# holoskii/Rendering

Hardware: AMD Instinct MI355X
Metric: Mrays/s + ms/frame at 4096^2, 250k-tri BVH scene (higher is better)
Workload: dtype f32

## Files before the change

include/rtx_debug.h:

```cpp
#ifndef RTX_DEBUG_H
#define RTX_DEBUG_H
#include "rtx.h"
#ifdef __cplusplus
extern "C" {
#endif

int rtx_frame_mode(rtx_scene* scene, int* mode, float* split_ms, float* fused_ms);
int rtx_set_frame_mode(rtx_scene* scene, int mode);

int rtx_mesh_flatten_probe(const rtx_mesh* mesh, uint32_t* n_wide, void* wide_out, void* prune_out, uint32_t cap_wide, float* root_rec8);
int rtx_wide_node_slots(void);

int rtx_frame_mode_probe(int forced, int has_list, int fused_gave_up, uint32_t listed, uint32_t rule_tiles, int warm, const uint32_t* frame_samples2,
                         const float* frame_ms2, uint32_t frames_seen, int* mode, int* reprobe, int* probing);

int rtx_tile_list_probe(uint32_t width, uint32_t height, uint32_t band_height, uint32_t n_parts, uint32_t part, int halo, uint32_t row_begin, uint32_t row_end,
                        int strips, const uint32_t* rect4, uint32_t* out, size_t cap, size_t* need);

int rtx_views_plan_probe(uint32_t n_views, const uint32_t* sizes2, uint32_t* items3_out, size_t cap_items, size_t* n_items);

int rtx_source_p_probe(const float* tris9, uint32_t n, const double* S3, double sigma, int cam, float* out);

int rtx_cost_grid_read(rtx_scene* scene, uint32_t* out, size_t n, uint32_t* grid_w, uint32_t* grid_h);

int rtx_set_knob(rtx_scene* scene, const char* name, double value);

#define RTX_VARIANT_BOXES    1u
#define RTX_VARIANT_PLAIN    2u
#define RTX_VARIANT_ANALYTIC 4u
#define RTX_VARIANT_STATS    8u
#define RTX_VARIANT_CULL     16u
int rtx_kernel_variant(rtx_scene* scene, uint32_t* bits);

int rtx_ssaa_list_read(rtx_scene* scene, uint32_t* info, uint32_t* scan, size_t n);

int rtx_kernel_time_reset(rtx_scene* scene);
int rtx_kernel_time_stats(rtx_scene* scene, int which, uint32_t* launches, double* total_ms);

int rtx_tile_cost_read(rtx_scene* scene, uint32_t* out, size_t n);

int rtx_math_probe(int device, int op, uint32_t n, const float* x, const float* y, float* out);

int rtx_vec_probe(int device, int op, uint32_t n, const float* a, const float* b, float ior, float* out);

int rtx_desc_serialize(const rtx_scene_desc* desc, void* out, size_t cap, size_t* need);

int rtx_bvh_build_mode(int mode);
int rtx_bvh_launches(const rtx_bvh* bvh, uint32_t* launches, int* queued);

int rtx_scene_mesh_read(rtx_scene* scene, uint32_t mesh, uint32_t* counts2, float* node_bounds, int32_t* node_skip, int32_t* leaf_begin,
                        int32_t* leaf_count, uint32_t* refs);
int rtx_scene_mesh_flat_read(rtx_scene* scene, uint32_t mesh, uint32_t* n_wide, void* wide_out, void* prune_out, uint32_t cap_wide, float* root_rec8);
int rtx_scene_edit_times(rtx_scene* scene, float* ms4);
int rtx_scene_lights_read(rtx_scene* scene, uint32_t* n_lights, rtx_light* lights_out, uint32_t cap_lights, size_t* n_point_floats,
                          float* points_out, size_t cap_point_floats);
int rtx_scene_mesh_prune_copy_read(rtx_scene* scene, uint32_t mesh, uint32_t copy, uint32_t* n_copies, uint32_t* n_wide, void* prune_out,
                                   uint32_t cap_wide);
int rtx_scene_objects_read(rtx_scene* scene, uint32_t* n_objects, rtx_object* objects_out, uint32_t cap_objects, uint32_t* n_meshes);

int rtx_live_device_memory(size_t* allocations, size_t* bytes);

struct rtx_mesh_topology;
struct rtx_mesh_pose;
int rtx_place_probe(int device, const struct rtx_mesh_topology* topology, const float* pos, const float* nrm, const struct rtx_mesh_pose* pose,
                    float* tri24_out, float* lo_hi_out, uint32_t* flags_out);

#ifdef __cplusplus
}
#endif
#endif
```

rendering_amd/__init__.py:

```python
import ctypes as C
import os

import numpy as np

HERE = os.path.dirname(os.path.abspath(__file__))
ROOT = os.path.dirname(HERE)
LIB_RTX = os.path.join(HERE, "librtx_hip.so")
LIB_HOST = os.path.join(HERE, "librendering_host.so")

__all__ = ["load", "Scene", "Comm", "RtxError", "device_count", "math_probe", "gather_plan", "exported_symbols", "sphere_directions", "cube_cameras"]


class RtxError(RuntimeError):
    pass


class Counters(C.Structure):
    _fields_ = [("rays", C.c_uint64), ("box_tests", C.c_uint64), ("tri_tests", C.c_uint64), ("moot_rays", C.c_uint64)]


_rtx = None
_host = None

RTX_SYMBOLS = [
    "rtx_last_error", "rtx_device_count", "rtx_scene_create", "rtx_scene_destroy", "rtx_scene_set_view", "rtx_scene_bytes",
    "rtx_render_pass1", "rtx_sobel", "rtx_render_ssaa", "rtx_render_frame", "rtx_render_ac", "rtx_frame_status", "rtx_frame_mode", "rtx_set_frame_mode", "rtx_set_knob", "rtx_cost_grid_read", "rtx_mesh_flatten_probe", "rtx_wide_node_slots", "rtx_source_p_probe", "rtx_quantize_bgr8", "rtx_render_frame_host",
    "rtx_counters_enable", "rtx_counters_reset", "rtx_counters_read", "rtx_last_kernel_ms", "rtx_math_probe",
    "rtx_cast_rays", "rtx_trace_rays", "rtx_kernel_time_reset", "rtx_kernel_time_stats", "rtx_tile_cost_read", "rtx_set_row_ownership",
    "rtx_bvh_build", "rtx_bvh_info", "rtx_bvh_read", "rtx_bvh_destroy",
    "rtx_vec_probe", "rtx_desc_serialize", "rtx_bvh_build_mode", "rtx_bvh_launches", "rtx_comm_unique_id", "rtx_comm_create", "rtx_comm_info", "rtx_comm_destroy", "rtx_comm_agree", "rtx_gather", "rtx_gather_plan",
    "rtx_scene_mesh_read", "rtx_scene_mesh_flat_read", "rtx_scene_edit_times", "rtx_kernel_variant", "rtx_ssaa_list_read", "rtx_live_device_memory",
    "rtx_scene_lights_read", "rtx_scene_mesh_prune_copy_read", "rtx_scene_objects_read",
    "rtx_frame_mode_probe", "rtx_tile_list_probe", "rtx_place_probe",
    "rtx_views_plan_probe",
]

RTX_EDIT_SYMBOLS = ["rtx_scene_set_object", "rtx_scene_update_mesh", "rtx_scene_set_lights", "rtx_scene_set_objects"]

RTX_QUERY_SYMBOLS = ["rtx_occluded_rays"]

RTX_AOV_SYMBOLS = ["rtx_render_aov"]


RTX_AO_SYMBOLS = ["rtx_render_ao"]

RTX_SURFACE_SYMBOLS = ["rtx_surface_rays"]

RTX_LIGHT_SYMBOLS = ["rtx_light_rays"]

RTX_SCATTER_SYMBOLS = ["rtx_scatter_rays", "rtx_sky_rays"]

RTX_POINTS_SYMBOLS = ["rtx_light_points", "rtx_ao_points"]

RTX_DEFORM_SYMBOLS = ["rtx_scene_set_mesh_topology", "rtx_scene_deform_mesh"]

RTX_VIEWS_SYMBOLS = ["rtx_render_views"]


class MeshTopology(C.Structure):
    _fields_ = [(n, C.c_uint32) for n in ("n_tris", "n_pos", "n_nrm", "n_uv", "placed_pos", "placed_nrm")] + \
               [(n, C.c_void_p) for n in ("corner_pos", "corner_nrm", "corner_uv", "uv", "nrm")]


class MeshPose(C.Structure):
    _fields_ = [("pos", C.c_float * 3), ("rot_matrix", C.c_float * 16), ("size", C.c_float * 3), ("bias", C.c_float), ("ac_penalty", C.c_int32)]


class AovBuffers(C.Structure):
    _fields_ = [(n, C.c_void_p) for n in ("depth_dev", "object_dev", "triangle_dev", "uv_dev", "normal_dev", "albedo_dev")]


class SurfaceBuffers(C.Structure):
    _fields_ = [(n, C.c_void_p) for n in ("hits_dev", "position_dev", "normal_dev", "albedo_dev", "specular_dev")]


class LightBuffers(C.Structure):
    _fields_ = [("n_lights", C.c_uint32)] + [(n, C.c_void_p) for n in ("hits_dev", "diffuse_dev", "specular_dev", "light_diffuse_dev",
                                                                       "light_specular_dev", "light_open_dev")]


class ScatterBuffers(C.Structure):
    _fields_ = [(n, C.c_void_p) for n in ("hits_dev", "local_dev", "reflect_dev", "refract_dev", "weight_dev", "kinds_dev")]


class ViewTarget(C.Structure):
    _fields_ = [("width", C.c_uint32), ("height", C.c_uint32), ("cam_pos", C.c_float * 3), ("cam_matrix", C.c_float * 16),
                ("scale", C.c_float), ("aspect", C.c_float), ("fb_dev", C.c_void_p), ("mask_dev", C.c_void_p)]


def cube_cameras(pos):
    p = tuple(float(x) for x in np.asarray(pos, np.float32).reshape(3))
    return [(p, rot, 90.0) for rot in ((0.0, 90.0, 0.0), (0.0, -90.0, 0.0), (-90.0, 0.0, 0.0), (90.0, 0.0, 0.0), (0.0, 180.0, 0.0), (0.0, 0.0, 0.0))]


def views_plan_probe(sizes):
    rtx, _ = load()
    sz = np.ascontiguousarray(np.asarray(sizes, np.uint32).reshape(-1, 2))
    n = C.c_size_t(0)
    _check(rtx.rtx_views_plan_probe(sz.shape[0], _np_ptr(sz), None, 0, C.byref(n)), "rtx_views_plan_probe")
    out = np.zeros((n.value, 3), np.uint32)
    _check(rtx.rtx_views_plan_probe(sz.shape[0], _np_ptr(sz), _np_ptr(out), n.value, C.byref(n)), "rtx_views_plan_probe")
    return out


class AoParams(C.Structure):
    _fields_ = [("n_dirs", C.c_uint32), ("dirs_dev", C.c_void_p), ("radius", C.c_float)]


def sphere_directions(n):
    n = int(n)
    if n < 2 or n % 2:
        raise ValueError("sphere_directions: n must be even and at least 2, got %d" % n)
    i = np.arange(n // 2, dtype=np.float64) + 0.5
    z = 1.0 - 2.0 * i / n
    phi = i * (np.pi * (3.0 - np.sqrt(5.0)))
    r = np.sqrt(1.0 - z * z)
    half = np.stack([r * np.cos(phi), r * np.sin(phi), z], 1).astype(np.float32)
    return np.concatenate([half, -half], 0)


def load():
    global _rtx, _host
    if _rtx is not None:
        return _rtx, _host
    for p in (LIB_RTX, LIB_HOST):
        if not os.path.exists(p):
            raise RtxError("native library %s is missing -- build it with ./build.sh (hipcc, gfx950); "
                           "there is no CPU fallback" % p)
    try:
        import torch
    except Exception:
        pass
    rtx = C.CDLL(LIB_RTX, mode=C.RTLD_GLOBAL)
    host = C.CDLL(LIB_HOST, mode=C.RTLD_GLOBAL)
    rtx.rtx_last_error.restype = C.c_char_p
    vp, u32, i32 = C.c_void_p, C.c_uint32, C.c_int
    rtx.rtx_device_count.argtypes = [C.POINTER(C.c_int)]
    rtx.rtx_render_pass1.argtypes = [vp, u32, u32, vp, vp]
    rtx.rtx_sobel.argtypes = [vp, vp, u32, u32, vp, vp]
    rtx.rtx_render_ssaa.argtypes = [vp, vp, u32, u32, vp, vp]
    rtx.rtx_render_frame.argtypes = [vp, u32, u32, vp, vp, vp]
    rtx.rtx_render_ac.argtypes = [vp, vp, vp, vp]
    rtx.rtx_frame_status.argtypes = [vp, C.POINTER(C.c_uint32)]
    rtx.rtx_set_frame_mode.argtypes = [vp, C.c_int]
    rtx.rtx_set_knob.argtypes = [vp, C.c_char_p, C.c_double]
    rtx.rtx_cost_grid_read.argtypes = [vp, vp, C.c_size_t, C.POINTER(C.c_uint32), C.POINTER(C.c_uint32)]
    rtx.rtx_mesh_flatten_probe.argtypes = [vp, C.POINTER(C.c_uint32), vp, vp, C.c_uint32, vp]
    rtx.rtx_source_p_probe.argtypes = [vp, u32, vp, C.c_double, i32, vp]
    rtx.rtx_frame_mode_probe.argtypes = [i32, i32, i32, u32, u32, i32, vp, vp, u32, C.POINTER(i32), C.POINTER(i32), C.POINTER(i32)]
    rtx.rtx_tile_list_probe.argtypes = [u32, u32, u32, u32, u32, i32, u32, u32, i32, vp, vp, C.c_size_t, C.POINTER(C.c_size_t)]
    rtx.rtx_frame_mode.argtypes = [vp, C.POINTER(C.c_int), C.POINTER(C.c_float), C.POINTER(C.c_float)]
    rtx.rtx_quantize_bgr8.argtypes = [vp, vp, vp, vp]
    rtx.rtx_render_frame_host.argtypes = [vp, i32, vp]
    rtx.rtx_counters_enable.argtypes = [vp, i32]
    rtx.rtx_counters_reset.argtypes = [vp]
    rtx.rtx_counters_read.argtypes = [vp, C.POINTER(Counters)]
    rtx.rtx_last_kernel_ms.argtypes = [vp, i32, C.POINTER(C.c_float)]
    rtx.rtx_math_probe.argtypes = [i32, i32, u32, vp, vp, vp]
    rtx.rtx_cast_rays.argtypes = [vp, u32, vp, vp, vp]
    rtx.rtx_trace_rays.argtypes = [vp, u32, vp, vp, vp, vp]
    rtx.rtx_occluded_rays.argtypes = [vp, u32, vp, vp, vp, vp]
    rtx.rtx_render_aov.argtypes = [vp, u32, u32, C.POINTER(AovBuffers), vp]
    rtx.rtx_render_ao.argtypes = [vp, u32, u32, C.POINTER(AoParams), vp, vp, vp]
    rtx.rtx_surface_rays.argtypes = [vp, u32, vp, C.POINTER(SurfaceBuffers), vp]
    if hasattr(rtx, "rtx_light_rays"):
        rtx.rtx_light_rays.argtypes = [vp, u32, vp, C.POINTER(LightBuffers), vp]
    if hasattr(rtx, "rtx_scatter_rays"):
        rtx.rtx_scatter_rays.argtypes = [vp, u32, vp, C.POINTER(ScatterBuffers), vp]
        rtx.rtx_sky_rays.argtypes = [vp, u32, vp, vp, vp]
    if hasattr(rtx, "rtx_light_points"):
        rtx.rtx_light_points.argtypes = [vp, u32, vp, vp, C.POINTER(LightBuffers), vp]
        rtx.rtx_ao_points.argtypes = [vp, u32, vp, C.POINTER(AoParams), vp, vp, vp]
    if hasattr(rtx, "rtx_render_views"):
        rtx.rtx_render_views.argtypes = [vp, u32, C.POINTER(ViewTarget), i32, vp]
        rtx.rtx_views_plan_probe.argtypes = [u32, vp, vp, C.c_size_t, C.POINTER(C.c_size_t)]
        host.rah_view_target.argtypes = [vp, vp, vp, C.c_float, i32, i32, C.POINTER(ViewTarget)]
    rtx.rtx_kernel_time_reset.argtypes = [vp]
    rtx.rtx_kernel_time_stats.argtypes = [vp, i32, C.POINTER(C.c_uint32), C.POINTER(C.c_double)]
    rtx.rtx_tile_cost_read.argtypes = [vp, vp, C.c_size_t]
    rtx.rtx_set_row_ownership.argtypes = [vp, u32, u32, u32, i32]
    rtx.rtx_bvh_build.argtypes = [vp, u32, vp, vp, C.c_int32, i32, C.POINTER(vp)]
    rtx.rtx_bvh_info.argtypes = [vp, C.POINTER(u32), C.POINTER(u32), C.POINTER(u32), C.POINTER(C.c_float)]
    rtx.rtx_bvh_launches.argtypes = [vp, C.POINTER(u32), C.POINTER(C.c_int)]
    rtx.rtx_bvh_read.argtypes = [vp, vp, vp, vp, vp, vp]
    rtx.rtx_bvh_destroy.argtypes = [vp]
    rtx.rtx_bvh_destroy.restype = None
    rtx.rtx_scene_bytes.argtypes = [vp, C.POINTER(C.c_size_t)]
    rtx.rtx_vec_probe.argtypes = [i32, i32, u32, vp, vp, C.c_float, vp]
    rtx.rtx_comm_unique_id.argtypes = [vp]
    rtx.rtx_comm_create.argtypes = [vp, i32, i32, i32, C.POINTER(vp)]
    rtx.rtx_comm_info.argtypes = [vp, C.POINTER(C.c_int), C.POINTER(C.c_int)]
    rtx.rtx_comm_destroy.argtypes = [vp]
    rtx.rtx_comm_agree.argtypes = [vp, C.c_int, C.POINTER(C.c_int), vp]
    rtx.rtx_comm_destroy.restype = None
    rtx.rtx_gather.argtypes = [vp, vp, vp, C.c_size_t, i32, i32, vp]
    rtx.rtx_gather_plan.argtypes = [u32, u32, u32, C.c_size_t, i32, u32, vp, vp, vp, C.POINTER(u32)]
    host.rah_set_ac_build.argtypes = [i32, i32]
    host.rah_set_ac_build.restype = None
    host.rah_set_ac_build_device.argtypes = [i32]
    host.rah_set_ac_build_device.restype = None
    host.rah_bvh_build_info.argtypes = [vp, i32, C.POINTER(C.c_int), C.POINTER(C.c_float)]
    host.rah_last_error.restype = C.c_char_p
    host.rah_scene_load.restype = vp
    host.rah_scene_load.argtypes = [C.c_char_p, C.c_char_p, i32, i32]
    host.rah_scene_free.argtypes = [vp]
    host.rah_scene_dims.argtypes = [vp] + [C.POINTER(C.c_int)] * 4
    host.rah_scene_resize.argtypes = [vp, i32, i32]
    host.rah_scene_set_device.argtypes = [vp, i32]
    host.rah_set_flag.argtypes = [vp, C.c_char_p, i32]
    host.rah_flatten.restype = vp
    host.rah_flatten.argtypes = [vp]
    host.rah_flat_desc.restype = vp
    host.rah_flat_desc.argtypes = [vp]
    host.rah_flat_free.argtypes = [vp]
    host.rah_bvh_counts.argtypes = [vp, i32, vp]
    host.rah_scene_gpu.restype = vp
    host.rah_scene_gpu.argtypes = [vp]
    host.rah_render_host.argtypes = [vp, vp, i32]
    host.rah_save_bmp.argtypes = [vp, vp, C.c_char_p]
    host.rah_bvh_dump.argtypes = [vp, i32, vp, vp, vp, vp, vp]
    host.rah_tris.argtypes = [vp, i32, vp]
    host.rah_camera.argtypes = [vp, vp, vp, vp, vp]
    host.rah_scene_digest.argtypes = [vp, vp, i32]
    host.rah_view_flags.argtypes = [vp]
    if hasattr(host, "rah_max_ray_depth"):
        host.rah_max_ray_depth.argtypes = [vp]
    host.rah_load_bmp.argtypes = [C.c_char_p, C.POINTER(C.c_int), C.POINTER(C.c_int), vp, i32]
    host.rah_object_move.argtypes = [vp, i32] + [vp] * 5
    host.rah_object_type.argtypes = [vp, i32]
    host.rah_object_move_times.argtypes = [vp, vp]
    rtx.rtx_scene_set_object.argtypes = [vp, C.c_uint32, vp]
    rtx.rtx_scene_update_mesh.argtypes = [vp, C.c_uint32, vp, vp, vp, vp, vp, i32, vp]
    rtx.rtx_scene_mesh_read.argtypes = [vp, C.c_uint32] + [vp] * 6
    rtx.rtx_scene_mesh_flat_read.argtypes = [vp, C.c_uint32, vp, vp, vp, C.c_uint32, vp]
    rtx.rtx_scene_edit_times.argtypes = [vp, vp]
    rtx.rtx_kernel_variant.argtypes = [vp, C.POINTER(C.c_uint32)]
    rtx.rtx_ssaa_list_read.argtypes = [vp, vp, vp, C.c_size_t]
    rtx.rtx_live_device_memory.argtypes = [C.POINTER(C.c_size_t), C.POINTER(C.c_size_t)]
    rtx.rtx_scene_set_lights.argtypes = [vp, C.c_uint32, vp]
    rtx.rtx_scene_lights_read.argtypes = [vp, C.POINTER(C.c_uint32), vp, C.c_uint32, C.POINTER(C.c_size_t), vp, C.c_size_t]
    rtx.rtx_scene_mesh_prune_copy_read.argtypes = [vp, C.c_uint32, C.c_uint32, C.POINTER(C.c_uint32), C.POINTER(C.c_uint32), vp, C.c_uint32]
# ... 220 lines not shown


class RtxView(C.Structure):
    _fields_ = [("width", C.c_uint32), ("height", C.c_uint32), ("bias", C.c_float), ("max_ray_depth", C.c_int32), ("background", C.c_float * 3),
                ("flags", C.c_uint32), ("cam_pos", C.c_float * 3), ("cam_matrix", C.c_float * 16), ("scale", C.c_float), ("aspect", C.c_float)]


class RtxSceneDesc(C.Structure):
    _fields_ = [("view", RtxView), ("n_objects", C.c_uint32), ("objects", C.POINTER(RtxObject)), ("n_meshes", C.c_uint32),
                ("meshes", C.POINTER(_RtxMesh)), ("n_lights", C.c_uint32), ("lights", C.POINTER(RtxLight)), ("sky_w", C.c_uint32), ("sky_h", C.c_uint32),
                ("sky", C.c_void_p * 6)]


class RtxMeshBuild(C.Structure):
    _fields_ = [("tri_pos_dev", C.c_void_p), ("tri_nrm_dev", C.c_void_p), ("tri_tb_dev", C.c_void_p), ("root_lo", C.c_float * 3),
                ("root_hi", C.c_float * 3), ("ac_penalty", C.c_int32)]


class RtxMeshSource(C.Structure):
    _fields_ = [("keep", C.c_int32), ("mesh", C.POINTER(_RtxMesh)), ("build", C.POINTER(RtxMeshBuild))]


def mesh_flatten_probe(bvh):
    rtx, _ = load()
    bounds = np.ascontiguousarray(bvh["bounds"], np.float32); skip = np.ascontiguousarray(bvh["skip"], np.int32)
    lb = np.ascontiguousarray(bvh["leaf_begin"], np.int32); lc = np.ascontiguousarray(bvh["leaf_count"], np.int32)
    refs = np.ascontiguousarray(bvh["refs"], np.uint32); pos = np.ascontiguousarray(bvh["tris"][:, 0:9], np.float32)
    m = _RtxMesh()
    m.n_nodes, m.n_refs, m.n_tris = len(skip), len(refs), len(pos)
    m.node_bounds, m.node_skip, m.leaf_begin, m.leaf_count = bounds.ctypes.data, skip.ctypes.data, lb.ctypes.data, lc.ctypes.data
    m.refs, m.tri_pos = refs.ctypes.data, pos.ctypes.data
    n = C.c_uint32(0)
    root = np.zeros(8, np.float32)
    _check(rtx.rtx_mesh_flatten_probe(C.byref(m), C.byref(n), None, None, 0, _np_ptr(root)), "rtx_mesh_flatten_probe")
    S = int(rtx.rtx_wide_node_slots())
    wide = np.zeros((n.value, S, 8), np.float32); prune = np.zeros((n.value, 2 * S, 8), np.float32)
    _check(rtx.rtx_mesh_flatten_probe(C.byref(m), C.byref(n), _np_ptr(wide), _np_ptr(prune), n.value, _np_ptr(root)), "rtx_mesh_flatten_probe")
    return wide, prune[:, 0:S], prune[:, S:2 * S], root


def source_p_probe(v0, e1, e2, S, sigma, cam):
    rtx, _ = load()
    t = np.ascontiguousarray(np.concatenate([v0, e1, e2], 1), np.float32)
    S = np.ascontiguousarray(S, np.float64)
    out = np.zeros(len(t), np.float32)
    _check(rtx.rtx_source_p_probe(_np_ptr(t), len(t), _np_ptr(S), float(sigma), 1 if cam else 0, _np_ptr(out)), "rtx_source_p_probe")
    return out


def frame_mode_probe(forced, has_list, fused_gave_up, listed, rule_tiles, warm, frame_samples, frame_ms, frames_seen):
    rtx, _ = load()
    n = np.ascontiguousarray(frame_samples, np.uint32); ms = np.ascontiguousarray(frame_ms, np.float32)
    assert n.shape == (2,) and ms.shape == (2,)
    mode, reprobe, probing = C.c_int(-1), C.c_int(-1), C.c_int(-1)
    _check(rtx.rtx_frame_mode_probe(int(forced), int(has_list), int(fused_gave_up), int(listed), int(rule_tiles), int(warm), _np_ptr(n), _np_ptr(ms),
                                    int(frames_seen), C.byref(mode), C.byref(reprobe), C.byref(probing)), "rtx_frame_mode_probe")
    return mode.value, bool(reprobe.value), bool(probing.value)


def tile_list_probe(width, height, ownership, rows, strips, rect):
    rtx, _ = load()
    r = np.ascontiguousarray(rect, np.uint32)
    assert r.shape == (4,)
    args = [int(width), int(height)] + [int(x) for x in ownership] + [int(rows[0]), int(rows[1]), 1 if strips else 0, _np_ptr(r)]
    need = C.c_size_t(0)
    _check(rtx.rtx_tile_list_probe(*args, None, 0, C.byref(need)), "rtx_tile_list_probe")
    out = np.zeros(need.value, np.uint32)
    _check(rtx.rtx_tile_list_probe(*args, _np_ptr(out), out.size, C.byref(need)), "rtx_tile_list_probe")
    return out


def math_probe(op, x, y=None, device=0):
    rtx, _ = load()
    x = np.ascontiguousarray(x, np.float32)
    out = np.zeros_like(x)
    yp = None
    if y is not None:
        y = np.ascontiguousarray(np.broadcast_to(np.asarray(y, np.float32), x.shape))
        yp = _np_ptr(y)
    _check(rtx.rtx_math_probe(device, op, x.size, _np_ptr(x), yp, _np_ptr(out)), "rtx_math_probe")
    return out


def vec_probe(op, a, b=None, ior=1.0, device=0):
    rtx, _ = load()
    a = np.ascontiguousarray(a, np.float32).reshape(-1, 3)
    out = np.zeros_like(a)
    bp = None
    if b is not None:
        b = np.ascontiguousarray(b, np.float32).reshape(-1, 3)
        bp = _np_ptr(b)
    _check(rtx.rtx_vec_probe(device, op, a.shape[0], _np_ptr(a), bp, ior, _np_ptr(out)), "rtx_vec_probe")
    return out


def euler_matrix(rot):
    _, host = load()
    r = np.ascontiguousarray(np.asarray(rot, np.float32).reshape(3))
    m = np.zeros((4, 4), np.float32)
    host.rah_euler_matrix(_np_ptr(r), _np_ptr(m))
    return m


def place_probe(topology, stored_normals, vertices, normals, pose, device=-1):
    rtx, _ = load()
    f32 = lambda a, cols: np.ascontiguousarray(np.asarray(a, np.float32).reshape(-1, cols))
    cp = np.ascontiguousarray(topology["corner_pos"], np.uint32).reshape(-1, 3)
    cn = np.ascontiguousarray(topology["corner_nrm"], np.int32).reshape(-1, 3)
    cu = np.ascontiguousarray(topology["corner_uv"], np.int32).reshape(-1, 3)
    uv, sn, P = f32(topology["uv"], 2), f32(stored_normals, 3), f32(vertices, 3)
    N = f32(normals, 3) if normals is not None else None
    if N is not None and N.shape != sn.shape:
        raise ValueError("place_probe: normals must have the stored normals' shape %s, got %s" % (sn.shape, N.shape))
    nt = cp.shape[0]
    t = MeshTopology(nt, P.shape[0], sn.shape[0], uv.shape[0], int(topology["placed_pos"]), int(topology["placed_nrm"]),
                     cp.ctypes.data, cn.ctypes.data, cu.ctypes.data, uv.ctypes.data if uv.size else None, sn.ctypes.data if sn.size else None)
    ps = MeshPose()
    ps.pos[:] = [float(x) for x in np.asarray(pose["pos"], np.float32)]
    ps.size[:] = [float(x) for x in np.asarray(pose["size"], np.float32)]
    ps.rot_matrix[:] = [float(x) for x in euler_matrix(pose["rot"]).reshape(-1)]
    ps.bias = float(pose["bias"]); ps.ac_penalty = int(pose["ac_penalty"])
    tri = np.zeros(max(nt, 1) * 24, np.float32)
    lo_hi = np.zeros(12, np.float32)
    flags = np.zeros(2, np.uint32)
    _check(rtx.rtx_place_probe(device, C.byref(t), _np_ptr(P), _np_ptr(N) if N is not None else None, C.byref(ps), _np_ptr(tri), _np_ptr(lo_hi), _np_ptr(flags)),
           "rtx_place_probe")
    return dict(pos=tri[:nt * 9].reshape(nt, 9).copy(), nrm=tri[nt * 9:nt * 18].reshape(nt, 9).copy(), tb=tri[nt * 18:nt * 24].reshape(nt, 6).copy(),
                obj_lo=lo_hi[0:3].copy(), obj_hi=lo_hi[3:6].copy(), root_lo=lo_hi[6:9].copy(), root_hi=lo_hi[9:12].copy(),
                bad_input=bool(flags[0]), bad_placed=bool(flags[1]))


class Scene:

    def __init__(self, scene_path, width=-1, height=-1, device=0, cwd=ROOT):
        self.rtx, self.host = load()
        self.host.rah_set_ac_build_device(device)
        self.h = C.c_void_p(self.host.rah_scene_load(cwd.encode(), scene_path.encode(), width, height))
        if not self.h:
            raise RtxError("could not load scene %s: %s" % (scene_path, self.host.rah_last_error().decode(errors="replace")))
        self.device = device
        self._cwd = cwd
        self.host.rah_scene_set_device(self.h, device)
        self._dims()
        self._gpu = None

    def _dims(self):
        w, h, no, nl = C.c_int(), C.c_int(), C.c_int(), C.c_int()
        self.host.rah_scene_dims(self.h, C.byref(w), C.byref(h), C.byref(no), C.byref(nl))
        self.width, self.height, self.n_objects, self.n_lights = w.value, h.value, no.value, nl.value

    def close(self):
        if self.h:
            self.host.rah_scene_free(self.h)
            self.h = None
            self._gpu = None

    def resize(self, width, height):
        self.host.rah_scene_resize(self.h, width, height)
        self._dims()

    def camera_pose(self):
        pos, rot = np.zeros(3, np.float32), np.zeros(3, np.float32)
        self.host.rah_camera_get.argtypes = [C.c_void_p] * 3
        self.host.rah_camera_get(self.h, _np_ptr(pos), _np_ptr(rot))
        return pos, rot

# ... 734 lines not shown
```

rendering_amd/csrc/rtx_api.hip:

```cpp
#include <hip/hip_runtime.h>

#include <cstdio>
#include <dlfcn.h>
#include <algorithm>
#include <array>
#include <functional>
#include <cmath>
#include <cstring>
#include <memory>
#include <string>
#include <type_traits>
#include <vector>

#include "../../include/rtx.h"
#include "../../include/rtx_debug.h"
#include "../../include/rtx_scene_edit.h"
#include "../../include/rtx_query.h"
#include "../../include/rtx_aov.h"
#include "../../include/rtx_ao.h"
#include "../../include/rtx_surface.h"
#include "../../include/rtx_light.h"
#include "../../include/rtx_scatter.h"
#include "../../include/rtx_points.h"
#include "../../include/rtx_views.h"
// ... 588 lines not shown
	HIPCHK(fixed.upload(m.diffuse_map, (size_t)m.diffuse_w * m.diffuse_h * 3, &dm.diffuse));
	HIPCHK(fixed.upload(m.normal_map, (size_t)m.normal_w * m.normal_h * 3, &dm.normal));
	HIPCHK(fixed.upload(m.specular_map, (size_t)m.specular_w * m.specular_h, &dm.specular));
	dm.dW = m.diffuse_w; dm.dH = m.diffuse_h; dm.nW = m.normal_w; dm.nH = m.normal_h; dm.sW = m.specular_w; dm.sH = m.specular_h;
	return RTX_OK;
}

int uploadMesh(rtx_scene* s, const rtx_mesh& m, uint32_t mi, uint32_t nLights, DevBag& owned, DevBag& fixed, Mesh& dm, rtx_scene::SrcMesh& sm,
               rtx_scene::MeshLeaves& leaves, float bounds[6])
{
	memset(&dm, 0, sizeof(dm));
	int rc;
	if ((rc = uploadMeshGeometry(s, m, mi, nLights, owned, dm, sm, leaves, bounds))) return rc;
	HIPCHK(owned.upload(m.tri_nrm, (size_t)m.n_tris * 9, &dm.nrm));
	HIPCHK(owned.upload(m.tri_tb, m.tri_tb ? (size_t)m.n_tris * 6 : 0, &dm.tb));
	return uploadMeshFixed(m, fixed, dm);
}

int checkObjects(uint32_t n, const rtx_object* objects, uint32_t nMeshes)
{
	if (n && !objects) return fail(RTX_ERR_ARG, "objects is NULL");
	for (uint32_t i = 0; i < n; i++) {
		const rtx_object& o = objects[i];
		if (o.type < RTX_OBJ_SPHERE || o.type > RTX_OBJ_MESH) return fail(RTX_ERR_ARG, "bad object type");
		if (o.material < 0 || o.material > 3) return fail(RTX_ERR_ARG, "bad material");
		if (o.type == RTX_OBJ_MESH && (o.mesh < 0 || (uint32_t)o.mesh >= nMeshes)) return fail(RTX_ERR_ARG, "bad mesh index");
	}
	return RTX_OK;
}

std::vector<Object> objectRecords(uint32_t n, const rtx_object* objects, const std::vector<Mesh>& meshes, const std::vector<rtx_scene::SrcMesh>& sms,
                                  const std::vector<float>& meshBounds)
{
	std::vector<Object> objs(n);
	for (uint32_t i = 0; i < n; i++) {
		const rtx_object& o = objects[i];
		Object& d = objs[i];
		memset(&d, 0, sizeof(d));
		d.type = o.type; d.material = o.material;
		memcpy(d.pos, o.pos, 12); memcpy(d.color, o.color, 12); memcpy(d.normal, o.normal, 12);
		d.ior = o.ior; d.ambient = o.ambient; d.diffuse = o.diffuse; d.specular = o.specular; d.nSpecular = o.n_specular;
		d.r2 = o.radius2; d.mesh = o.mesh;
		if (o.type == RTX_OBJ_MESH) meshObjectRecord(&meshBounds[(size_t)o.mesh * 6], d, meshes[o.mesh], sms[o.mesh]);
	}
	return objs;
}

int uploadRecords(const std::vector<Mesh>& meshes, const std::vector<Object>& objs, const std::vector<float>& sb, DevBag& bag, const Mesh** devMeshes,
                  const Object** devObjs, const float** devSpheres)
{
	HIPCHK(bag.upload(sb.data(), sb.size(), devSpheres));
	HIPCHK(bag.upload(meshes.data(), meshes.size(), devMeshes));
	HIPCHK(bag.upload(objs.data(), objs.size(), devObjs));
	return RTX_OK;
}

void chooseAnalytic(rtx_scene* s)
{
	s->analytic = true;
	for (const Object& d : s->objectRecs) if (d.type == RTX_OBJ_MESH) s->analytic = false;
}

int checkLights(uint32_t n, const rtx_light* lights)
{
	if (n && !lights) return fail(RTX_ERR_ARG, "lights is NULL");
	for (uint32_t i = 0; i < n; i++) {
		const rtx_light& l = lights[i];
		if (l.type < RTX_LIGHT_DISTANT || l.type > RTX_LIGHT_AREA) return fail(RTX_ERR_ARG, "bad light type");
		if (l.type == RTX_LIGHT_AREA && (!l.points || l.n_points == 0)) return fail(RTX_ERR_ARG, "area light without sample points");
	}
	return RTX_OK;
}

int uploadLights(uint32_t n, const rtx_light* lights, DevBag& bag, std::vector<Light>& recs, const Light** dev)
{
	recs.resize(n);
	for (uint32_t i = 0; i < n; i++) {
		const rtx_light& l = lights[i];
		Light& d = recs[i];
		memset(&d, 0, sizeof(d));
		d.type = l.type; memcpy(d.color, l.color, 12); d.intensity = l.intensity;
		memcpy(d.dir, l.dir, 12); memcpy(d.pos, l.pos, 12);
		d.nPoints = l.n_points;
		if (l.type == RTX_LIGHT_AREA) HIPCHK(bag.upload(l.points, (size_t)l.n_points * 3, &d.points));
	}
	HIPCHK(bag.upload(recs.data(), recs.size(), dev));
	return RTX_OK;
}

void deriveLights(rtx_scene* s, uint32_t n, const rtx_light* lights)
{
	s->srcLightPos.clear(); s->srcLightIsPoint.clear(); s->estLights.clear();
	for (uint32_t i = 0; i < n; i++) {
		const rtx_light& l = lights[i];
		s->srcLightPos.push_back({ { l.pos[0], l.pos[1], l.pos[2] } });
		s->srcLightIsPoint.push_back(l.type == RTX_LIGHT_POINT ? 1 : 0);
		if (l.type == RTX_LIGHT_POINT) s->estLights.push_back({ { l.pos[0], l.pos[1], l.pos[2], 2.0f } });
		else if (l.type == RTX_LIGHT_DISTANT) s->estLights.push_back({ { l.dir[0], l.dir[1], l.dir[2], 1.0f } });
		else if (l.type == RTX_LIGHT_AREA) s->estLights.push_back({ { l.pos[0], l.pos[1], l.pos[2], 2.0f + 4.0f * (float)std::min<uint32_t>(l.n_points, 4096u) } });
	}
	s->params.nLights = n;
	s->params.nSrcLights = s->knobs.sources ? std::min<uint32_t>(n, kMaxSrcLights) : 0u;
}

void choosePlain(rtx_scene* s)
{
	s->plain = true;
	for (const Object& d : s->objectRecs) if (d.material != 0) s->plain = false;
	for (const Light& l : s->lightRecs) if (l.type == RTX_LIGHT_AREA) s->plain = false;
}

std::vector<float> analyticEstimate(rtx_scene* s, const rtx_object* objects, size_t n)
{
	std::vector<float> sb;
	s->estPlanes.clear();
	s->srcNmax = 1.0f;
	for (size_t i = 0; i < n; i++) {
		const rtx_object& o = objects[i];
		if (o.type == RTX_OBJ_PLANE) {
			s->estPlanes.push_back({ { o.pos[0], o.pos[1], o.pos[2], o.normal[0], o.normal[1], o.normal[2] } });
			const double nl = std::sqrt((double)o.normal[0] * o.normal[0] + (double)o.normal[1] * o.normal[1] + (double)o.normal[2] * o.normal[2]);
			if (!(nl <= 1e30)) s->srcNmax = INFINITY; else s->srcNmax = std::max(s->srcNmax, (float)(nl * 1.000001));
		}
		if (o.type != RTX_OBJ_SPHERE || !(o.radius2 > 0) || !std::isfinite(o.radius2)) continue;
		const float r = std::sqrt(o.radius2), w = (o.material == 1 || o.material == 2) ? 4000.0f : 300.0f;
		sb.insert(sb.end(), { o.pos[0] - r, o.pos[1] - r, o.pos[2] - r, o.pos[0] + r, o.pos[1] + r, o.pos[2] + r, w, 0.0f });
	}
	s->params.srcNmax2 = s->srcNmax * s->srcNmax * 1.00001f;
	return sb;
}

}

extern "C" {

const char* rtx_last_error(void) { return gErr.c_str(); }

int rtx_device_count(int* count)
{
	if (!count) return fail(RTX_ERR_ARG, "count is NULL");
	*count = 0;
	int n = 0;
	hipError_t e = hipGetDeviceCount(&n);
	if (e != hipSuccess) return fail(RTX_ERR_NO_DEVICE, std::string("hipGetDeviceCount: ") + hipGetErrorString(e));
	*count = n;
	return RTX_OK;
}

int rtx_scene_create(const rtx_scene_desc* desc, int device, rtx_scene** out)
{
	if (!desc || !out) return fail(RTX_ERR_ARG, "desc/out is NULL");
	*out = nullptr;
	int n = 0;
	if (hipGetDeviceCount(&n) != hipSuccess || n <= 0) return fail(RTX_ERR_NO_DEVICE, "no HIP device visible");
	if (device < 0 || device >= n) return fail(RTX_ERR_ARG, "device index out of range");
	HIPCHK(hipSetDevice(device));
	hipDeviceProp_t prop;
	HIPCHK(hipGetDeviceProperties(&prop, device));

	std::unique_ptr<rtx_scene, void (*)(rtx_scene*)> hold(new rtx_scene, rtx_scene_destroy);
	rtx_scene* s = hold.get();
	readKnobs(s->knobs);
	s->tileQueues.reserve(16);
	s->device = device;
	s->numCUs = prop.multiProcessorCount;
	memset(&s->params, 0, sizeof(Params));
// ... 1358 lines not shown

int rtx_views_plan_probe(uint32_t n_views, const uint32_t* sizes2, uint32_t* items3_out, size_t cap_items, size_t* n_items)
{
	if (!n_items || (n_views && !sizes2)) return fail(RTX_ERR_ARG, "rtx_views_plan_probe: NULL argument");
	uint64_t items = 0;
	if (int rc = checkViewSizes(n_views, sizes2, sizes2 + 1, 8, &items)) return rc;
	*n_items = (size_t)items;
	if (!items3_out || cap_items < items) return RTX_OK;
	std::vector<uint32_t> first(n_views + 1, 0u);
	for (uint32_t v = 0; v < n_views; v++) first[v + 1] = first[v] + (uint32_t)rtxviews::tilesOf(sizes2[2 * v], sizes2[2 * v + 1]);
	for (uint32_t item = 0; item < (uint32_t)items; item++) {
		const uint32_t v = rtxviews::viewOfItem([&](uint32_t i) { return first[i]; }, n_views, item);
		const rtxviews::Tile t = rtxviews::tileOfItem(item, first[v], rtxviews::tilesAcross(sizes2[2 * v]));
		items3_out[3 * (size_t)item] = v; items3_out[3 * (size_t)item + 1] = t.tx; items3_out[3 * (size_t)item + 2] = t.ty;
	}
	return RTX_OK;
}

int rtx_render_views(rtx_scene* s, uint32_t n_views, const rtx_view_target* views, int with_ssaa, void* stream)
{
	RoctxRange range("Render views (rtx_render_views)");
	if (!s) return fail(RTX_ERR_ARG, "scene is NULL");
	if (n_views == 0) return RTX_OK;
	if (!views) return fail(RTX_ERR_ARG, "rtx_render_views: views is NULL");
	uint64_t items64 = 0;
	if (int rc = checkViewSizes(n_views, &views[0].width, &views[0].height, sizeof(rtx_view_target), &items64)) return rc;
	for (uint32_t i = 0; i < n_views; i++) {
		if (!views[i].fb_dev) return fail(RTX_ERR_ARG, "rtx_render_views: view " + std::to_string(i) + " has no framebuffer (fb_dev is NULL)");
		if (with_ssaa && !views[i].mask_dev) return fail(RTX_ERR_ARG, "rtx_render_views: view " + std::to_string(i) + " has no mask (mask_dev is NULL) and SSAA is asked for");
	}
	if (s->params.bandH && s->params.nParts > 1) return fail(RTX_ERR_ARG, "rtx_render_views: the rows are shared among devices (rtx_set_row_ownership); deal out views, not rows");
	if (s->stats) return fail(RTX_ERR_UNSUPPORTED, "rtx_render_views collects no statistics (rtx_counters_enable)");
	if (showNormals(s)) return fail(RTX_ERR_UNSUPPORTED, "rtx_render_views does not render the normals view (RTX_FLAG_SHOW_NORMALS)");
	const uint32_t nItems = (uint32_t)items64;
	int rc = ensureWork(s);
	if (rc) return rc;
	hipStream_t st = (hipStream_t)stream;
	if ((rc = renderOn(s, st))) return rc;
	const size_t recBytes = (size_t)n_views * sizeof(ViewRec), tableBytes = recBytes + ((size_t)n_views + 1) * sizeof(uint32_t);
	HIPCHK(s->viewsTable.reserve(tableBytes));
	HIPCHK(s->viewsWork.reserve(64));
	if (with_ssaa) { HIPCHK(s->viewsItemView.reserve(nItems)); HIPCHK(s->viewsList.reserve((size_t)nItems * 64)); }
	if (s->viewsStagePending) { HIPCHK(hipEventSynchronize(s->viewsStaged)); s->viewsStagePending = false; }
	HIPCHK(s->viewsStage.reserve(tableBytes));
	ViewRec* recs = (ViewRec*)s->viewsStage.host();
	uint32_t* first = (uint32_t*)(s->viewsStage.host() + recBytes);
	uint32_t at = 0;
	for (uint32_t i = 0; i < n_views; i++) {
		const rtx_view_target& t = views[i];
		ViewRec& r = recs[i];
		r.width = t.width; r.height = t.height; r.scale = t.scale; r.aspect = t.aspect;
		memcpy(r.camPos, t.cam_pos, 12); memcpy(r.camM, t.cam_matrix, 64);
		r.firstItem = first[i] = at;
		r.fb = t.fb_dev; r.mask = t.mask_dev;
		r.tilesX = rtxviews::tilesAcross(t.width); r.pad[0] = r.pad[1] = r.pad[2] = 0;
		at += (uint32_t)rtxviews::tilesOf(t.width, t.height);
	}
	first[n_views] = at;
	HIPCHK(hipMemcpyAsync(s->viewsTable.get(), s->viewsStage.host(), tableBytes, hipMemcpyHostToDevice, st));
	HIPCHK(s->viewsStaged.create(hipEventDisableTiming));
	HIPCHK(hipEventRecord(s->viewsStaged, st));
	s->viewsStagePending = true;
	HIPCHK(hipMemsetAsync(s->viewsWork.get(), 0, 64 * sizeof(uint32_t), st));
	ViewsKernArgs k;
	k.P = s->params;
	k.A.views = (const ViewRec*)s->viewsTable.get(); k.A.first = (const uint32_t*)(s->viewsTable.get() + recBytes);
	k.A.nViews = n_views; k.A.nItems = nItems;
	k.A.itemView = s->viewsItemView; k.A.list = s->viewsList; k.A.heads = s->viewsWork;
	const Variant v = variantOf(s);
	const uint32_t itemBlocks = (nItems + 3) / 4;
	hipLaunchKernelGGL(viewsPass1Kernel(v), dim3(std::min<uint32_t>((uint32_t)s->blocksPass1, itemBlocks)), dim3(256), 0, st, k);
	HIPCHK(hipGetLastError());
	if (!with_ssaa) return RTX_OK;
	hipLaunchKernelGGL(rtxViewsMaskKernel, dim3(itemBlocks), dim3(256), 0, st, k.A);
	HIPCHK(hipGetLastError());
	k.P.frames = s->frames + s->framesArea;
	hipLaunchKernelGGL(viewsSsaaKernel(v), dim3(std::min<uint32_t>((uint32_t)s->blocksSsaa, nItems)), dim3(256), 0, st, k);
	HIPCHK(hipGetLastError());
	return RTX_OK;
}

int rtx_math_probe(int device, int op, uint32_t n, const float* x, const float* y, float* out)
{
	if (!x || !out || op < 0 || op > 4) return fail(RTX_ERR_ARG, "bad argument");
	int cnt = 0;
	if (hipGetDeviceCount(&cnt) != hipSuccess || cnt <= 0) return fail(RTX_ERR_NO_DEVICE, "no HIP device visible");
	HIPCHK(hipSetDevice(device));
	DevArray<float> dx, dy, dout;
	const size_t bytes = (size_t)n * sizeof(float);
	HIPCHK(dx.reserve(n)); HIPCHK(dy.reserve(n)); HIPCHK(dout.reserve(n));
	HIPCHK(hipMemcpy(dx, x, bytes, hipMemcpyHostToDevice));
	if (y) HIPCHK(hipMemcpy(dy, y, bytes, hipMemcpyHostToDevice));
	else HIPCHK(hipMemset(dy, 0, bytes));
	hipLaunchKernelGGL(rtxMathProbeKernel, dim3((n + 255) / 256), dim3(256), 0, nullptr, op, n, (const float*)dx, (const float*)dy, dout.get());
	HIPCHK(hipGetLastError());
	HIPCHK(hipMemcpy(out, dout, bytes, hipMemcpyDeviceToHost));
	return RTX_OK;
}

int rtx_vec_probe(int device, int op, uint32_t n, const float* a, const float* b, float ior, float* out)
{
	if (!a || !out || op < 0 || op > 3 || (op < 3 && !b)) return fail(RTX_ERR_ARG, "bad argument");
	int cnt = 0;
	if (hipGetDeviceCount(&cnt) != hipSuccess || cnt <= 0) return fail(RTX_ERR_NO_DEVICE, "no HIP device visible");
	HIPCHK(hipSetDevice(device));
	DevArray<float> da, db, dout;
	const size_t bytes = (size_t)n * 3 * sizeof(float);
	HIPCHK(da.reserve((size_t)n * 3)); HIPCHK(dout.reserve((size_t)n * 3));
	HIPCHK(hipMemcpy(da, a, bytes, hipMemcpyHostToDevice));
	if (b) { HIPCHK(db.reserve((size_t)n * 3)); HIPCHK(hipMemcpy(db, b, bytes, hipMemcpyHostToDevice)); }
	hipLaunchKernelGGL(rtxVecProbeKernel, dim3((n + 255) / 256), dim3(256), 0, nullptr, op, n, (const float*)da, (const float*)db, ior, dout.get());
	HIPCHK(hipGetLastError());
	HIPCHK(hipMemcpy(out, dout, bytes, hipMemcpyDeviceToHost));
	return RTX_OK;
}

}

#include "rtx_comm.hip"

#include "rtx_edit.hip"

#include "rtx_deform.hip"
```

rendering_amd/csrc/rtx_device.h:

```cpp
#pragma once
#include <stdint.h>

namespace rtxd {

struct Node {
	float b[6];
	int32_t link;
	int32_t first;
};
static_assert(sizeof(Node) == 32, "node must be one s_load_dwordx8");

constexpr int kWideLevels = 3;
constexpr int kWideSlots = 1 << kWideLevels;
constexpr int kWideStackEntries = 72;
struct WideNode { Node slot[kWideSlots]; };
static_assert(kWideSlots == 8 && sizeof(WideNode) == 32 * kWideSlots, "wide node = eight slots, two s_load_dwordx16 per four");

struct RefA { float v0x, v0y, v0z; uint32_t tri; };
struct RefB { float e1x, e1y, e1z, e2x; };
struct RefC { float e2y, e2z; };
static_assert(sizeof(RefA) == 16 && sizeof(RefB) == 16 && sizeof(RefC) == 8, "reference records = dwordx4 + dwordx4 + dwordx2");

struct PruneRec { float c[3]; float P; float h[3]; float Pgen; };
static_assert(sizeof(PruneRec) == 32, "prune record = two dwordx4");
constexpr uint32_t kMaxSrcLights = 6;
constexpr float kSrcAinfMax = 32.0f;
struct PlaneRec { float qc[3]; float wlo; float qr[3]; float whi; };
static_assert(sizeof(PlaneRec) == 32, "plane record = two dwordx4");
struct PruneBlock { PruneRec box[kWideSlots]; PlaneRec plane[kWideSlots]; };
static_assert(sizeof(PruneBlock) == 64 * kWideSlots, "prune block");

struct Mesh {
	const Node* nodes;
	const RefA* refA;
	const RefB* refB;
	const RefC* refC;
	const float* nrm;
	const float* uv;
	const float* tb;
	const float* diffuse;
	const float* normal;
	const float* specular;
	uint32_t nNodes, nRefs, nTris;
	uint32_t dW, dH, nW, nH, sW, sH;
	uint32_t boxesRegular;
	const struct WideNode* wide;
	uint32_t nWide, padw;
	const PruneBlock* prune;
	float vmax, padv;
	PruneRec rootRec;
	float fatRadius, centre[3], radius;
};

struct Object {
	int32_t type, material;
	float pos[3];
	float r2;
	float normal[3];
	int32_t mesh;
	float color[3];
	float ior, ambient, diffuse, specular, nSpecular;
	float rootBox[6];
	float fatRadius, centre[3], radius;
	uint32_t meshFlags;
	uint32_t pad[2];
	const Node* nodes; const RefA* refA; const RefB* refB; const RefC* refC; const struct WideNode* wide; const struct PruneBlock* prune;
	uint32_t nNodes; float vmax;
	uint32_t pruneBoxes;
	uint32_t srcStride;
};
static_assert(sizeof(Object) == 192, "object record = three 64-byte lines");

struct Light {
	int32_t type;
	float color[3];
	float intensity;
	float dir[3];
	float pos[3];
	uint32_t nPoints;
	const float* points;
	uint32_t pad[2];
};
static_assert(sizeof(Light) == 64, "light record = one 64-byte line");

struct View {
	uint32_t width, height;
	float bias;
	int32_t maxDepth;
	float bg[3];
	uint32_t flags;
	float camPos[3];
	float camM[16];
	float scale, aspect;
};

struct Params {
	View view;
	const Object* objects;
	const Mesh* meshes;
	const Light* lights;
	const float* const* sky;
	uint32_t nObjects, nLights, skyW, skyH;
	uint32_t rowBegin, rowEnd;
	uint32_t tilesX, tileRow0, nTiles;
	uint32_t bandH, nParts, part, halo;
	uint32_t* workCounter;
	const uint32_t* tileList;
	uint32_t tilesY, pad3;
	const uint8_t* ssaaMask;
	const uint32_t* ssaaPixels;
	const uint32_t* ssaaScan;
	uint32_t* tileCost;
	uint32_t tilesXFull, pad2;
	float* frames;
	uint32_t totalLanes;
	uint32_t nSrcLights;
	float* fb;
	const float* probeRays;
	float* probeHits;
	float* probeColours;
	uint32_t nProbe;
	float srcNmax2;
	unsigned long long* counters;
	uint32_t* tileReady;
	uint32_t* tileSobel;
	const uint8_t* tileNeed;
	unsigned long long* tileFlags;
	unsigned long long* ssaaQueue;
	unsigned long long* frameCtl;
	const uint32_t* countExpect;
	const uint32_t* splitLimits;
	uint8_t* maskOut;
	uint32_t listedTiles, epoch, queueCap, veryBudget, tilesYFull, heavyTicks, stripBit, padF1;
};

constexpr int kFrameFields = 14;

}
```

rendering_amd/csrc/rtx_kernels.hip:

```cpp
#include <hip/hip_runtime.h>
#include <stdint.h>

#include "rtx_device.h"
#include "rtx_tuning.h"

#pragma clang fp contract(off)

using namespace rtxd;

constexpr uint32_t kPopNum = 1u, kPopDen = 2u;

namespace {

#if RTX_DBG
#define RTX_DBG_ONLY(...) __VA_ARGS__
#else
#define RTX_DBG_ONLY(...)
#endif
#if RTX_DBG || RTX_WAVE_TRACE
#define RTX_TRACE_ONLY(...) __VA_ARGS__
#else
#define RTX_TRACE_ONLY(...)
#endif

// ... 199 lines not shown
	uint64_t ki = (uint64_t)__double_as_longlong(kd);
	kd -= 0x1.8p+47;
	double rr = ylogx - kd;
	uint64_t t = powTab[32 + ki % 32];
	t += (ki + signBias) << (52 - 5);
	double s = __longlong_as_double((long long)t);
	double zz = __builtin_fma(0x1.c6af84b912394p-5, rr, 0x1.ebfce50fac4f3p-3);
	double rr2 = rr * rr;
	double yv = __builtin_fma(0x1.62e42ff0c52d6p-1, rr, 1.0);
	yv = __builtin_fma(zz, rr2, yv);
	yv = yv * s;
	return (float)yv;
}

__device__ __forceinline__ V3 reflectDir(V3 d, V3 n) { float k = 2 * dot(d, n); return d - n * k; }

__device__ __forceinline__ V3 refractDir(V3 d, V3 n, float ior)
{
	float n1 = 1, n2 = ior;
	float cosi = clampRef(-1, 1, dot(d, n));
	V3 mn = n;
	if (cosi < 0) cosi = -cosi;
	else { float t = n1; n1 = n2; n2 = t; mn = -n; }
	float rri = n1 / n2;
	float k = 1 - rri * rri * (1 - cosi * cosi);
	if (k < 0) return mk(0, 0, 0);
	return d * rri + mn * (rri * cosi - __builtin_sqrtf(k));
}

__device__ __forceinline__ float fresnelKr(V3 d, V3 n, float ior)
{
	float n1 = 1, n2 = ior;
	float cosi = clampRef(-1, 1, dot(d, n));
	if (cosi > 0) { float t = n1; n1 = n2; n2 = t; }
	float sint = n1 / n2 * __builtin_sqrtf(fmaxRef(0.f, 1 - cosi * cosi));
	if (sint >= 1) return 1;
	float cost = __builtin_sqrtf(fmaxRef(0.f, 1 - sint * sint));
	cosi = fabsf(cosi);
	float rs = ((n2 * cosi) - (n1 * cost)) / ((n2 * cosi) + (n1 * cost));
	float rp = ((n1 * cosi) - (n2 * cost)) / ((n1 * cosi) + (n2 * cost));
	return (rs * rs + rp * rp) / 2;
}

__device__ __forceinline__ int toPixel(float v, int mx)
{
	int val = (int)((v + 1.0f) / 2.0f * mx);
	if (val >= mx) val = mx - 1;
	if (val < 0) val = 0;
	return val;
}
__device__ __forceinline__ V3 load3(const float* p) { return mk(p[0], p[1], p[2]); }
typedef const __attribute__((address_space(1))) float* GlobalFloats;
__device__ __forceinline__ GlobalFloats inGlobal(const float* p) { return (GlobalFloats)(uintptr_t)p; }
__device__ __forceinline__ V3 load3(GlobalFloats p) { return mk(p[0], p[1], p[2]); }

__device__ __noinline__ V3 skyFetch(const float* const* sky, int W, int H, V3 dir)
{
	float ax = fabsf(dir.x), ay = fabsf(dir.y), az = fabsf(dir.z);
	float m = fmaxRef(ax, fmaxRef(ay, az));
	V3 a; int face, i, j;
	if (m == az) {
		if (dir.z < 0) { a = dir * (1 / -dir.z); face = 1; i = toPixel(a.y, H); j = toPixel(a.x, W); }
		else { a = dir * (1 / dir.z); face = 3; i = toPixel(a.y, H); j = toPixel(-a.x, W); }
	}
	else if (m == ax) {
		if (dir.x < 0) { a = dir * (1 / -dir.x); face = 0; i = toPixel(a.y, H); j = toPixel(-a.z, W); }
		else { a = dir * (1 / dir.x); face = 2; i = toPixel(a.y, H); j = toPixel(a.z, W); }
	}
	else {
		if (dir.y < 0) { a = dir * (1 / -dir.y); face = 5; i = toPixel(a.z, H); j = toPixel(a.x, W); }
		else { a = dir * (1 / dir.y); face = 4; i = toPixel(a.z, H); j = toPixel(a.x, W); }
	}
	return load3(inGlobal(sky[face]) + ((size_t)i * W + j) * 3);
}

__device__ __forceinline__ V3 skyColor(const Params& P, V3 dir)
{
	if (!(P.view.flags & 2u)) return mk(P.view.bg[0], P.view.bg[1], P.view.bg[2]);
	return skyFetch(P.sky, (int)P.skyW, (int)P.skyH, dir);
}

__device__ __forceinline__ int texel(int dim, float coord) { int v = (int)(dim * coord); if (v >= dim) v = dim - 1; if (v < 0) v = 0; return v; }

__device__ __forceinline__ float attenuation(float intensity, float l2)
{
	return fminRef(1.0f, (float)((double)intensity / (4 * 3.14159265358979323846 * (double)l2 / 1000)));
}

struct Hit { int obj; float t; uint32_t tri; float u, v; };
RTX_TRACE_ONLY(__device__ unsigned long long gDbgWave[3 * 16384];)
RTX_DBG_ONLY(
__device__ unsigned long long gDbgTimeline[3 * 8192 * 160];
__device__ unsigned long long gDbgHist[64];
)
#if RTX_DBG >= 3
#define RTX_T0 const unsigned long long dbgB0 = __builtin_readcyclecounter();
#define RTX_ACC(k) { const unsigned long long dbgE = __builtin_readcyclecounter() - dbgB0; if (__lane_id() == (uint32_t)__ffsll((long long)ballot(true)) - 1u) { atomicAdd(&gDbgHist[16 + 2 * (k)], dbgE); atomicAdd(&gDbgHist[17 + 2 * (k)], 1ull); } }
#else
#define RTX_T0
#define RTX_ACC(k)
#endif
struct Counts { unsigned long long rays, box, tri, wNodes, wTri, wS2, wS3, wS4, wLeaves, wLeafSkips, wChunks, wChunkSkips, triLanes, moot, cNodes, cFilter, cExact,
                aWalks, sWalks, sVisits, sLeaves, sPasses, sExact; };

template <typename T> __device__ __forceinline__ T after(T x, uint32_t v)
{
	asm("" : "+s"(x) : "s"(v));
	return x;
}

__device__ __forceinline__ float waveMax(float v)
{
#define RTX_STEP(ctrl) "s_nop 1\n\tv_max_f32_dpp %0, %0, %0 " ctrl "\n\t"
	asm volatile(RTX_STEP("quad_perm:[1,0,3,2] row_mask:0xf bank_mask:0xf") RTX_STEP("quad_perm:[2,3,0,1] row_mask:0xf bank_mask:0xf")
	             RTX_STEP("row_half_mirror row_mask:0xf bank_mask:0xf") RTX_STEP("row_mirror row_mask:0xf bank_mask:0xf")
	             RTX_STEP("row_bcast:15 row_mask:0xa bank_mask:0xf") RTX_STEP("row_bcast:31 row_mask:0xc bank_mask:0xf")
	             "s_nop 0" : "+v"(v));
#undef RTX_STEP
	return __int_as_float(__builtin_amdgcn_readlane(__float_as_int(v), 63));
}

struct Bundle {
	float ocx, ocy, ocz, rox, roy, roz;
	float dcx, dcy, dcz, rdx, rdy, rdz;
	float kd;
	float roMax;
	float kdRoSum;
	float roRd;
	bool sane;
};
constexpr float kFilterK = 0x1p-18f;
constexpr float kFilterEta = 1e-30f;

__device__ __forceinline__ void centreRadius(float lo, float hi, float& c, float& r)
{
	c = unif(0.5f * (lo + hi));
	r = unif((0.5f * (hi - lo)) * (1.0f + 0x1p-19f) + 0x1p-21f * fmaxf(fabsf(lo), fabsf(hi)));
}

__device__ __forceinline__ void waveMaxMin(float v, float& hi, float& lo)
{
#define RTX_STEP(ctrl) "v_max_f32_dpp %0, %0, %0 " ctrl "\n\tv_min_f32_dpp %1, %1, %1 " ctrl "\n\ts_nop 0\n\t"
	asm volatile("s_nop 1\n\t"
		"v_max_f32_dpp %0, %2, %2 quad_perm:[1,0,3,2] row_mask:0xf bank_mask:0xf\n\tv_min_f32_dpp %1, %2, %2 quad_perm:[1,0,3,2] row_mask:0xf bank_mask:0xf\n\ts_nop 0\n\t"
		RTX_STEP("quad_perm:[2,3,0,1] row_mask:0xf bank_mask:0xf")
		RTX_STEP("row_half_mirror row_mask:0xf bank_mask:0xf") RTX_STEP("row_mirror row_mask:0xf bank_mask:0xf")
		RTX_STEP("row_bcast:15 row_mask:0xa bank_mask:0xf") RTX_STEP("row_bcast:31 row_mask:0xc bank_mask:0xf")
		"s_nop 0" : "=&v"(hi), "=&v"(lo) : "v"(v));
#undef RTX_STEP
	hi = __int_as_float(__builtin_amdgcn_readlane(__float_as_int(hi), 63));
	lo = __int_as_float(__builtin_amdgcn_readlane(__float_as_int(lo), 63));
}

__device__ __forceinline__ Bundle makeBundle(bool active, const V3& o, const V3& d, bool sameOrigin = false)
{
	const float qnan = __builtin_nanf("");
	Bundle B;
	float lo, hi;
#define RTX_RANGE(x, c, r) waveMaxMin(active ? (x) : qnan, hi, lo); centreRadius(lo, hi, c, r)
	if (sameOrigin) {
		const int first = __builtin_ctzll(ballot(active) | (1ull << 63));
		B.ocx = __int_as_float(__builtin_amdgcn_readlane(__float_as_int(o.x), first)); B.ocy = __int_as_float(__builtin_amdgcn_readlane(__float_as_int(o.y), first));
		B.ocz = __int_as_float(__builtin_amdgcn_readlane(__float_as_int(o.z), first));
		B.rox = B.roy = B.roz = 0.0f;
	}
	else {
		RTX_RANGE(o.x, B.ocx, B.rox); RTX_RANGE(o.y, B.ocy, B.roy); RTX_RANGE(o.z, B.ocz, B.roz);
	}
	RTX_RANGE(d.x, B.dcx, B.rdx); RTX_RANGE(d.y, B.dcy, B.rdy); RTX_RANGE(d.z, B.dcz, B.rdz);
// ... 48 lines not shown
	const float ax = B.ocx - ra.v0x, ay = B.ocy - ra.v0y, az = B.ocz - ra.v0z;
	const float s1 = fabsf(e1x) + fabsf(e1y) + fabsf(e1z), s2 = fabsf(e2x) + fabsf(e2y) + fabsf(e2z);
	const float wux = __builtin_fmaf(e2y, az, -(e2z * ay)), wuy = __builtin_fmaf(e2z, ax, -(e2x * az)), wuz = __builtin_fmaf(e2x, ay, -(e2y * ax));
	float nuc = __builtin_fmaf(B.dcz, wuz, __builtin_fmaf(B.dcy, wuy, B.dcx * wux));
	const float cux = __builtin_fmaf(B.dcy, e2z, -(B.dcz * e2y)), cuy = __builtin_fmaf(B.dcz, e2x, -(B.dcx * e2z)), cuz = __builtin_fmaf(B.dcx, e2y, -(B.dcy * e2x));
	const float nurO = __builtin_fmaf(B.roRd, s2, __builtin_fmaf(B.roz, fabsf(cuz), __builtin_fmaf(B.roy, fabsf(cuy), B.rox * fabsf(cux))));
	const float nur = (nurO + __builtin_fmaf(B.rdz, fabsf(wuz), __builtin_fmaf(B.rdy, fabsf(wuy), B.rdx * fabsf(wux)))) * (1.0f + 0x1p-19f);
	const float Eu = __builtin_fmaf(f.kda, s2, kFilterEta);
	if (!CULL) nuc *= f.sg;
	const float nuLo = nuc - nur - Eu;
	const uint64_t rejU = (ballot(nuc + nur < -Eu) | ballot(nuLo > f.detHi1)) & f.ok;
	if ((open & ~rejU) == 0) return rejU;
	const float wvx = __builtin_fmaf(ay, e1z, -(az * e1y)), wvy = __builtin_fmaf(az, e1x, -(ax * e1z)), wvz = __builtin_fmaf(ax, e1y, -(ay * e1x));
	float nvc = __builtin_fmaf(B.dcz, wvz, __builtin_fmaf(B.dcy, wvy, B.dcx * wvx));
	const float cvx = __builtin_fmaf(e1y, B.dcz, -(e1z * B.dcy)), cvy = __builtin_fmaf(e1z, B.dcx, -(e1x * B.dcz)), cvz = __builtin_fmaf(e1x, B.dcy, -(e1y * B.dcx));
	const float nvrO = __builtin_fmaf(B.roRd, s1, __builtin_fmaf(B.roz, fabsf(cvz), __builtin_fmaf(B.roy, fabsf(cvy), B.rox * fabsf(cvx))));
	const float nvr = (nvrO + __builtin_fmaf(B.rdz, fabsf(wvz), __builtin_fmaf(B.rdy, fabsf(wvy), B.rdx * fabsf(wvx)))) * (1.0f + 0x1p-19f);
	const float Ev = __builtin_fmaf(f.kda, s1, kFilterEta);
	if (!CULL) nvc *= f.sg;
	return rejU | ((ballot(nvc + nvr < -Ev) | ballot(nuLo + (nvc - nvr - Ev) > f.detHi1)) & f.ok);
}

template <bool CULL, bool STATS>
__device__ __forceinline__ void triTestOne(float v0x, float v0y, float v0z, float e1x, float e1y, float e1z, float e2x, float e2y, float e2z,
                                           uint32_t tri, const V3& o, const V3& d, float& bt, float& bu, float& bv, uint32_t& btri)
{
	const float px = d.y * e2z - d.z * e2y, py = d.z * e2x - d.x * e2z, pz = d.x * e2y - d.y * e2x;
	const float det = e1x * px + e1y * py + e1z * pz;
	if ((CULL ? det : fabsf(det)) < RTX_EPS8) return;
	const float tx = o.x - v0x, ty = o.y - v0y, tz = o.z - v0z;
	const float nu = tx * px + ty * py + tz * pz;
	if (CULL) {
		if (nu < -0x1p-20f || nu > det * (1.0f + 0x1p-20f)) return;
	}
	const float inv = 1 / det;
	const float u = nu * inv;
	if (u < 0 || u > 1) return;
	const float qx = ty * e1z - tz * e1y, qy = tz * e1x - tx * e1z, qz = tx * e1y - ty * e1x;
	const float v = (d.x * qx + d.y * qy + d.z * qz) * inv;
	if (v < 0 || u + v > 1) return;
	const float t = (e2x * qx + e2y * qy + e2z * qz) * inv;
	if (t < 0) return;
	if (t < bt) { bt = t; bu = u; bv = v; btri = tri; }
}

template <bool CULL>
__device__ __forceinline__ void triTestLane(const RefA& ra, const RefB& rb, const RefC& rc, float ox, float oy, float oz, float dx, float dy, float dz,
                                            float& t, float& u, float& v)
{
	const float e1x = rb.e1x, e1y = rb.e1y, e1z = rb.e1z, e2x = rb.e2x, e2y = rc.e2y, e2z = rc.e2z;
	const float px = dy * e2z - dz * e2y, py = dz * e2x - dx * e2z, pz = dx * e2y - dy * e2x;
	const float det = e1x * px + e1y * py + e1z * pz;
	if ((CULL ? det : fabsf(det)) < RTX_EPS8) return;
	const float tx = ox - ra.v0x, ty = oy - ra.v0y, tz = oz - ra.v0z;
	const float nu = tx * px + ty * py + tz * pz;
	if (CULL) { if (nu < -0x1p-20f || nu > det * (1.0f + 0x1p-20f)) return; }
	const float inv = 1 / det;
	const float uu = nu * inv;
	if (uu < 0 || uu > 1) return;
	const float qx = ty * e1z - tz * e1y, qy = tz * e1x - tx * e1z, qz = tx * e1y - ty * e1x;
	const float vv = (dx * qx + dy * qy + dz * qz) * inv;
	if (vv < 0 || uu + vv > 1) return;
	const float tt = (e2x * qx + e2y * qy + e2z * qz) * inv;
	if (tt < 0) return;
	t = tt; u = uu; v = vv;
}

#define RTX_LEAF_BATCH_MAX (RTX_LEAF_BATCH > RTX_LEAF_BATCH_FEW ? RTX_LEAF_BATCH : RTX_LEAF_BATCH_FEW)
struct LeafEntry { uint32_t start, count, first, pad0, maskLo, maskHi, pad1, pad2; };
typedef uint32_t u32x4v __attribute__((ext_vector_type(4)));
__shared__ LeafEntry leafBatch[4][RTX_LEAF_BATCH_MAX];
struct WideItem { int32_t link; uint32_t first, maskLo, maskHi; };
__shared__ WideItem wideStack[4][kWideStackEntries];
__shared__ float pruneUni[4][48];
constexpr float kPruneC = 216.0f;
__device__ __forceinline__ bool boxFailsRegular(float blox, float bhix, float bloy, float bhiy, float bloz, float bhiz, const V3& o, float ix, float iy, float iz)
{
	const float xlo = (blox - o.x) * ix, xhi = (bhix - o.x) * ix, ylo = (bloy - o.y) * iy, yhi = (bhiy - o.y) * iy;
	const float zlo = (bloz - o.z) * iz, zhi = (bhiz - o.z) * iz;
	float nx, ny, nz, fx, fy, fz, tn, tf;
	asm("v_min_f32 %0, %1, %2" : "=v"(nx) : "v"(xlo), "v"(xhi)); asm("v_max_f32 %0, %1, %2" : "=v"(fx) : "v"(xlo), "v"(xhi));
	asm("v_min_f32 %0, %1, %2" : "=v"(ny) : "v"(ylo), "v"(yhi)); asm("v_max_f32 %0, %1, %2" : "=v"(fy) : "v"(ylo), "v"(yhi));
	asm("v_min_f32 %0, %1, %2" : "=v"(nz) : "v"(zlo), "v"(zhi)); asm("v_max_f32 %0, %1, %2" : "=v"(fz) : "v"(zlo), "v"(zhi));
	asm("v_max3_f32 %0, %1, %2, %3" : "=v"(tn) : "v"(nx), "v"(ny), "v"(nz));
	asm("v_min3_f32 %0, %1, %2, %3" : "=v"(tf) : "v"(fx), "v"(fy), "v"(fz));
	return tn > tf;
}

__device__ __forceinline__ uint32_t pruneLaneK(const float* pu)
{
	const uint32_t lane = laneNow(), axis = lane & 3u;
	const uint32_t word = 2u * lane - axis;
	uint32_t ui = (lane >> 5) * 3u + axis;
	ui = ui < 5u ? ui : 5u;
	const uint32_t lds = (uint32_t)(uintptr_t)(const __attribute__((address_space(3))) float*)(pu + ui * 8u);
	return lds << 16 | word * 4u;
}
template <bool BOXES, bool CULL = true>
__device__ __forceinline__ uint32_t pruneEval8(const RTX_AS1 char* blk, const float* pu, float tmaxB, uint32_t laneK = 0)
{
	static_assert(kWideSlots == 8, "pruneEval8: lanes = 16 records x 4");
	const uint32_t off = laneK & 0xffffu;
	const float f0 = *(const RTX_AS1 float*)(blk + off), f1 = *(const RTX_AS1 float*)(blk + off + 16u);
	const __attribute__((address_space(3))) f4v* ur = (const __attribute__((address_space(3))) f4v*)(uintptr_t)(laneK >> 16);
	const f4v ua = ur[0], ub = ur[1];
	const float c = __uint_as_float(__float_as_uint(f0) ^ __float_as_uint(ub.x));
	const float ai = fmaxf(c - ua.z, ua.w - c) + f1;
	const float ax = fabsf(f0) + f1;
	const float dq = __builtin_fmaf(ua.y, ax, __builtin_fmaf(fabsf(ua.x), f1, ua.x * f0));
	const float oq = ua.z * f0;
	const float orr = __builtin_fmaf(ua.w, ax, fabsf(ua.z) * f1);
	const float pm = oq - orr, pp = oq + orr;
	float ainf, dqHi, oqLo, oqHi, w0, w1, t0, t1, t2, t3;
	asm volatile("s_nop 1\n\t"
	             "v_max_f32_dpp %6, %10, %10 quad_perm:[1,2,0,3] row_mask:0xf bank_mask:0xf\n\t"
	             "v_add_f32_dpp %7, %11, %11 quad_perm:[1,2,0,3] row_mask:0xf bank_mask:0xf\n\t"
	             "v_add_f32_dpp %8, %12, %12 quad_perm:[1,2,0,3] row_mask:0xf bank_mask:0xf\n\t"
	             "v_add_f32_dpp %9, %13, %13 quad_perm:[1,2,0,3] row_mask:0xf bank_mask:0xf\n\t"
	             "v_mov_b32_dpp %4, %14 quad_perm:[3,3,3,3] row_mask:0xf bank_mask:0xf\n\t"
	             "v_mov_b32_dpp %5, %15 quad_perm:[3,3,3,3] row_mask:0xf bank_mask:0xf\n\t"
	             "v_max_f32_dpp %0, %10, %6 quad_perm:[2,0,1,3] row_mask:0xf bank_mask:0xf\n\t"
	             "v_add_f32_dpp %1, %11, %7 quad_perm:[2,0,1,3] row_mask:0xf bank_mask:0xf\n\t"
	             "v_add_f32_dpp %2, %12, %8 quad_perm:[2,0,1,3] row_mask:0xf bank_mask:0xf\n\t"
	             "v_add_f32_dpp %3, %13, %9 quad_perm:[2,0,1,3] row_mask:0xf bank_mask:0xf"
	             : "=&v"(ainf), "=&v"(dqHi), "=&v"(oqLo), "=&v"(oqHi), "=&v"(w0), "=&v"(w1), "=&v"(t0), "=&v"(t1), "=&v"(t2), "=&v"(t3)
	             : "v"(ai), "v"(dq), "v"(pm), "v"(pp), "v"(f0), "v"(f1));
	const float detHi = dqHi + ub.x;
	const float ntHi = (w1 - oqLo) + ub.y, ntLo = (w0 - oqHi) - ub.y;
	uint64_t deadPlane;
	if (CULL) deadPlane = ballot(detHi < 0.0f) | ballot(ntHi < 0.0f) | (ballot(detHi > 0.0f) & ballot(ntLo >= tmaxB * (detHi * (1.0f + 0x1p-18f))));
	else {
		const float dql = __builtin_fmaf(-ua.y, ax, __builtin_fmaf(-fabsf(ua.x), f1, ua.x * f0));
		float dqLo;
		asm volatile("s_nop 1\n\t"
		             "v_add_f32_dpp %1, %2, %2 quad_perm:[1,2,0,3] row_mask:0xf bank_mask:0xf\n\t"
		             "s_nop 1\n\t"
		             "v_add_f32_dpp %0, %2, %1 quad_perm:[2,0,1,3] row_mask:0xf bank_mask:0xf"
		             : "=&v"(dqLo), "=&v"(t0) : "v"(dql));
		const float detLo = dqLo - ub.x;
		const uint64_t front = ballot(detLo > 0.0f), back = ballot(detHi < 0.0f);
		deadPlane = (front & (ballot(ntHi < 0.0f) | ballot(ntLo >= tmaxB * (detHi * (1.0f + 0x1p-18f))))) |
		            (back & (ballot(ntLo > 0.0f) | ballot(-ntHi >= tmaxB * (-detLo * (1.0f + 0x1p-18f)))));
	}
	uint32_t deadBits = (uint32_t)(deadPlane >> 32);
	if (BOXES) {
		const float Pn = ainf <= kSrcAinfMax ? w0 : w1;
		const float rho = __builtin_fmaf(ub.z * ainf, Pn, 0x1p-17f * (ainf + ub.w)) * (1.0f + 0x1p-20f) + 1e-30f;
		const float hh = f1 + rho;
		const float a = (c - hh) - ua.w, b = (c + hh) - ua.z;
		const float e = fminf(fminf(a * ua.x, a * ua.y), ub.y), f = fmaxf(fmaxf(b * ua.x, b * ua.y), -ub.y);
		float ent, ext;
		asm volatile("s_nop 1\n\t"
		             "v_max_f32_dpp %2, %4, %4 quad_perm:[1,2,0,3] row_mask:0xf bank_mask:0xf\n\t"
		             "v_min_f32_dpp %3, %5, %5 quad_perm:[1,2,0,3] row_mask:0xf bank_mask:0xf\n\t"
		             "s_nop 0\n\t"
		             "v_max_f32_dpp %0, %4, %2 quad_perm:[2,0,1,3] row_mask:0xf bank_mask:0xf\n\t"
		             "v_min_f32_dpp %1, %5, %3 quad_perm:[2,0,1,3] row_mask:0xf bank_mask:0xf"
		             : "=&v"(ent), "=&v"(ext), "=&v"(t0), "=&v"(t1) : "v"(e), "v"(f));
		const uint64_t deadBox = ballot(ent > ext) | ballot(ext < 0.0f) | ballot(ent > tmaxB * (1.0f + 0x1p-18f));
		deadBits |= (uint32_t)deadBox;
	}
	return ~deadBits & 0x11111111u;
}

template <bool STATS, bool CULL, bool REGULAR, bool WIDE = false, bool FEWRAYS = false, bool BOXES = true>
__device__ __forceinline__ void meshWalk(const u32x16& mp, const Bundle& B, bool consider, bool shadow, const V3& o, const V3& d,
                                         float ix, float iy, float iz, bool sx, bool sy, bool sz, float tLimit,
                                         float& bt, float& bu, float& bv, uint32_t& btri, Counts& cnt, uint32_t srcSel = 0)
{
#define RTX_MP(k) (((uint64_t)mp[2 * (k) + 1] << 32) | mp[2 * (k)])
	const Node* nodes = (const Node*)RTX_MP(0);
	const RTX_AS1 char* refA = (const RTX_AS1 char*)(uintptr_t)RTX_MP(1);
	const RTX_AS1 char* refB = (const RTX_AS1 char*)(uintptr_t)RTX_MP(2);
	const RTX_AS1 char* refC = (const RTX_AS1 char*)(uintptr_t)RTX_MP(3);
	const uint32_t nN = mp[12];
	bt = kFltMax; bu = 0; bv = 0; btri = 0;
	if (nN == 0) return;
	constexpr uint32_t kLeafBatch = FEWRAYS ? RTX_LEAF_BATCH_FEW : RTX_LEAF_BATCH;
	float tmaxB = unif(waveMax(consider ? tLimit : -__builtin_inff()));
	uint32_t resume = consider ? 0u : kNever;
	const uint32_t nRays4 = 4u * (uint32_t)__popcll(ballot(consider));
	uint32_t i = 0;
	const uint32_t last = nN - 1;
	u32x8 nd = sload8(nodes);
	LeafEntry* entries = leafBatch[threadIdx.x >> 6];
	WideItem* stack = wideStack[threadIdx.x >> 6];
	const WideNode* wideNodes = WIDE ? (const WideNode*)RTX_MP(4) : nullptr;
	uint32_t sp = 0;
	const RTX_AS1 char* pruneRecs = nullptr;
	float* pu = pruneUni[threadIdx.x >> 6];
	if (WIDE) {
		pruneRecs = (const RTX_AS1 char*)(uintptr_t)RTX_MP(5);
#undef RTX_MP
		if (pruneRecs != nullptr) {
			pruneRecs += (size_t)srcSel * mp[15] * sizeof(PruneBlock);
			const float dlx = B.dcx - B.rdx, dhx = B.dcx + B.rdx, dly = B.dcy - B.rdy, dhy = B.dcy + B.rdy, dlz = B.dcz - B.rdz, dhz = B.dcz + B.rdz;
			const float wide = 1.0f + 0x1p-21f, narrow = 1.0f - 0x1p-21f;
			float lx = __builtin_amdgcn_rcpf(dhx), hx = __builtin_amdgcn_rcpf(dlx);
			float ly = __builtin_amdgcn_rcpf(dhy), hy = __builtin_amdgcn_rcpf(dly), lz = __builtin_amdgcn_rcpf(dhz), hz = __builtin_amdgcn_rcpf(dlz);
			lx *= lx > 0 ? narrow : wide; hx *= hx > 0 ? wide : narrow;
			ly *= ly > 0 ? narrow : wide; hy *= hy > 0 ? wide : narrow;
			lz *= lz > 0 ? narrow : wide; hz *= hz > 0 ? wide : narrow;
			const bool usx = (dlx > 0x1p-100f || dhx < -0x1p-100f), usy = (dly > 0x1p-100f || dhy < -0x1p-100f), usz = (dlz > 0x1p-100f || dhz < -0x1p-100f);
			if (laneNow() == 0) {
				const bool nx = hx < 0, ny = hy < 0, nz = hz < 0;
				const bool okx = usx && (lx > 0 || nx), oky = usy && (ly > 0 || ny), okz = usz && (lz > 0 || nz);
				const float ilx = nx ? -hx : lx, ihx = nx ? -lx : hx, ily = ny ? -hy : ly, ihy = ny ? -ly : hy, ilz = nz ? -hz : lz, ihz = nz ? -lz : hz;
				const float ocx = nx ? -B.ocx : B.ocx, ocy = ny ? -B.ocy : B.ocy, ocz = nz ? -B.ocz : B.ocz;
				const float cap = B.kd * (kPruneC / kFilterK);
				const float omax = fmaxf(fmaxf(fabsf(B.ocx) + B.rox, fabsf(B.ocy) + B.roy), fabsf(B.ocz) + B.roz);
				const float eB = kFilterK * (omax + F(mp[13])) * (1.0f + 0x1p-20f) + 1e-30f;
				const float inf = __builtin_inff(), kd2 = 2.0f * B.kd;
				*(f4v*)(pu + 0) = f4v{ ilx, ihx, ocx - B.rox, ocx + B.rox };  *(f4v*)(pu + 4) = f4v{ __uint_as_float(nx ? 0x80000000u : 0u), okx ? inf : -inf, cap, omax };
				*(f4v*)(pu + 8) = f4v{ ily, ihy, ocy - B.roy, ocy + B.roy };  *(f4v*)(pu + 12) = f4v{ __uint_as_float(ny ? 0x80000000u : 0u), oky ? inf : -inf, cap, omax };
				*(f4v*)(pu + 16) = f4v{ ilz, ihz, ocz - B.roz, ocz + B.roz }; *(f4v*)(pu + 20) = f4v{ __uint_as_float(nz ? 0x80000000u : 0u), okz ? inf : -inf, cap, omax };
				float dcx = B.dcx, dcy = B.dcy, dcz = B.dcz, rdx = B.rdx, rdy = B.rdy, rdz = B.rdz;
				asm volatile("" : "+v"(dcx), "+v"(dcy), "+v"(dcz), "+v"(rdx), "+v"(rdy), "+v"(rdz));
				*(f4v*)(pu + 24) = f4v{ dcx, rdx, B.ocx, B.rox }; *(f4v*)(pu + 28) = f4v{ kd2, eB, 0.0f, 0.0f };
				*(f4v*)(pu + 32) = f4v{ dcy, rdy, B.ocy, B.roy }; *(f4v*)(pu + 36) = f4v{ kd2, eB, 0.0f, 0.0f };
				*(f4v*)(pu + 40) = f4v{ dcz, rdz, B.ocz, B.roz }; *(f4v*)(pu + 44) = f4v{ kd2, eB, 0.0f, 0.0f };
			}
			if (!B.sane) pruneRecs = nullptr;
		}
	}
	if (WIDE && RTX_DBG) { cnt.aWalks++; if (shadow) cnt.sWalks++; }
	uint32_t laneK = WIDE ? pruneLaneK(pu) : 0u;
	asm volatile("" : "+v"(laneK));
	if (WIDE) {
		const uint64_t m0 = ballot(consider);
		if (laneNow() == 0) { WideItem it; it.link = 1; it.first = 0; it.maskLo = (uint32_t)m0; it.maskHi = (uint32_t)(m0 >> 32); stack[0] = it; }
		sp = 1;
	}
	for (;;) {
		RTX_DBG_ONLY(const unsigned long long dbgP1 = __builtin_readcyclecounter();)
		uint32_t batch = 0, total = 0;
		uint32_t soleFirst = 0;
		uint32_t myReach = 0;
		if (WIDE) {
			const uint32_t lane = laneNow();
			const uint64_t openM = ballot(resume != kNever);
			auto noteLeaf = [&](int32_t link, uint32_t first, uint64_t m) {
				const bool in = ((((lane & 32u) ? (uint32_t)(m >> 32) : (uint32_t)m) >> (lane & 31u)) & 1u) != 0;
				const uint32_t n = (uint32_t)~link;
				if (RTX_DBG) { cnt.wLeaves++; if (shadow) cnt.sLeaves++; }
				if (m != 0 && n != 0) {
					if (kLeafBatch == 1 && !FEWRAYS) soleFirst = uni(first);
					else if (lane == 0) {
						LeafEntry en;
						en.first = first; en.count = n; en.maskLo = (uint32_t)m; en.maskHi = (uint32_t)(m >> 32); en.start = total; en.pad0 = en.pad1 = en.pad2 = 0;
						entries[batch] = en;
					}
					myReach |= in ? 1u << batch : 0u;
					batch = uni(batch + 1);
					total = uni(total + n);
				}
			};
#define RTX_PUSH(lnk, fst, m)                                                                                                  \
			{                                                                                                                  \
				if (lane == 0) { WideItem ni; ni.link = (int32_t)(lnk); ni.first = (fst); ni.maskLo = (uint32_t)(m); ni.maskHi = (uint32_t)((m) >> 32); stack[sp] = ni; } \
				sp = uni(sp + 1);                                                                                              \
			}
			while (sp != 0 && batch < kLeafBatch) {
				sp = uni(sp - 1);
				const WideItem it = stack[sp];
				const int32_t link = (int32_t)uni((uint32_t)it.link);
				const uint32_t itFirst = it.first;
				const uint32_t mlo = uni(it.maskLo), mhi = uni(it.maskHi);
				const uint64_t inM = ((uint64_t)mhi << 32 | mlo) & openM;
				if (link < 0) {
					noteLeaf(link, itFirst, inM);
					continue;
				}
				if (inM == 0) continue;
				if (RTX_DBG) { cnt.wNodes++; if (shadow) cnt.sVisits++; }
				const WideNode* w = wideNodes + (uint32_t)(link - 1);
				u32x16 wa = sload16(w), wb = sload16((const char*)w + 64);
				uint32_t aliveM = 0x11111111u;
				const bool evalPrune = pruneRecs != nullptr;
				if (evalPrune) {
					aliveM = pruneEval8<BOXES, CULL>(pruneRecs + ((size_t)(uint32_t)(link - 1) << 9), pu, tmaxB, laneK);
					if (RTX_DBG) { cnt.wS4++; cnt.wLeafSkips += (uint32_t)kWideSlots - (uint32_t)__popc(aliveM); }
				}
#define RTX_ALIVE(k) ((aliveM >> (4 * (k))) & 1u)
#define RTX_ALIVE4(q) ((aliveM >> (16 * (q))) & 0x1111u)
#define RTX_SLOT(rec, base, k)                                                                                                     \
				if ((int32_t)rec[base + 6] != 0 && RTX_ALIVE(k)) {                                                         \
					const bool fail = boxFailsRegular(F(rec[base]), F(rec[base + 1]), F(rec[base + 2]), F(rec[base + 3]), F(rec[base + 4]), F(rec[base + 5]), o, ix, iy, iz); \
					const uint64_t mk_ = ballot(!fail) & inM;                                                                       \
					if (RTX_DBG) cnt.wS3++;                                                                                         \
					if (mk_ != 0) RTX_PUSH(rec[base + 6], rec[base + 7], mk_)                                                       \
				}
				if (RTX_ALIVE4(1) != 0) {
#pragma unroll
					for (int q4 = kWideSlots / 4 - 1; q4 >= 1; --q4) {
						if (RTX_ALIVE4(q4) == 0) continue;
						const u32x16 wc = sload16((const char*)w + 128 * q4), wd = sload16((const char*)w + 128 * q4 + 64);
						RTX_SLOT(wd, 8, 4 * q4 + 3) RTX_SLOT(wd, 0, 4 * q4 + 2) RTX_SLOT(wc, 8, 4 * q4 + 1) RTX_SLOT(wc, 0, 4 * q4)
					}
					const char* w0 = (const char*)w;
					asm volatile("" : "+s"(w0));
					wa = sload16(w0); wb = sload16(w0 + 64);
				}
				if (RTX_ALIVE4(0) != 0) {
					RTX_SLOT(wb, 8, 3) RTX_SLOT(wb, 0, 2) RTX_SLOT(wa, 8, 1)
					if ((int32_t)wa[6] != 0 && RTX_ALIVE(0)) {
						const bool fail = boxFailsRegular(F(wa[0]), F(wa[1]), F(wa[2]), F(wa[3]), F(wa[4]), F(wa[5]), o, ix, iy, iz);
						const uint64_t mk_ = ballot(!fail) & inM;
						if (RTX_DBG) cnt.wS3++;
						if (mk_ != 0) {
							if ((int32_t)wa[6] < 0 && batch < kLeafBatch) noteLeaf((int32_t)wa[6], wa[7], mk_);
							else RTX_PUSH(wa[6], wa[7], mk_)
						}
					}
				}
#undef RTX_SLOT
#undef RTX_PUSH
#undef RTX_ALIVE
#undef RTX_ALIVE4
			}
		}
		else {
			while (i < nN && batch < kLeafBatch) {
				const int32_t link = (int32_t)nd[6];
				const uint32_t next = uni(i + 1);
				const uint32_t nxt = link > 0 ? (uint32_t)link : next;
				const Node* nb = after(nodes, nd[7]);
				const u32x8 nxA = sload8(nb + (next < last ? next : last));
				const u32x8 nxB = sload8(nb + (nxt < last ? nxt : last));
				const bool act = i >= resume;
				const float xlo = (F(nd[0]) - o.x) * ix, xhi = (F(nd[1]) - o.x) * ix, ylo = (F(nd[2]) - o.y) * iy, yhi = (F(nd[3]) - o.y) * iy;
				const float zlo = (F(nd[4]) - o.z) * iz, zhi = (F(nd[5]) - o.z) * iz;
				bool fail;
				if (REGULAR) {
					float nx, ny, nz, fx, fy, fz, tn, tf;
					asm("v_min_f32 %0, %1, %2" : "=v"(nx) : "v"(xlo), "v"(xhi)); asm("v_max_f32 %0, %1, %2" : "=v"(fx) : "v"(xlo), "v"(xhi));
					asm("v_min_f32 %0, %1, %2" : "=v"(ny) : "v"(ylo), "v"(yhi)); asm("v_max_f32 %0, %1, %2" : "=v"(fy) : "v"(ylo), "v"(yhi));
					asm("v_min_f32 %0, %1, %2" : "=v"(nz) : "v"(zlo), "v"(zhi)); asm("v_max_f32 %0, %1, %2" : "=v"(fz) : "v"(zlo), "v"(zhi));
					asm("v_max3_f32 %0, %1, %2, %3" : "=v"(tn) : "v"(nx), "v"(ny), "v"(nz));
					asm("v_min3_f32 %0, %1, %2, %3" : "=v"(tf) : "v"(fx), "v"(fy), "v"(fz));
					fail = tn > tf;
				}
				else {
					float tmin = sx ? xhi : xlo, tmx = sx ? xlo : xhi;
					const float tymin = sy ? yhi : ylo, tymax = sy ? ylo : yhi;
					fail = (tmin > tymax) || (tymin > tmx);
					if (tymin > tmin) tmin = tymin;
					if (tymax < tmx) tmx = tymax;
					const float tzmin = sz ? zhi : zlo, tzmax = sz ? zlo : zhi;
					fail = fail || (tmin > tzmax) || (tzmin > tmx);
				}
				const bool pass = act && !fail;
				if (act && fail) resume = nxt;
				if (STATS) cnt.box += __popcll(ballot(act));
				if (RTX_DBG) cnt.wNodes++;
				const uint64_t m = ballot(pass);
				if (m == 0) {
					nd = nxB;
					i = uni(nxt);
					continue;
				}
				if (link < 0) {
					const uint32_t n = (uint32_t)~link;
					if (STATS) cnt.tri += (unsigned long long)__popcll(m) * n;
					if (RTX_DBG) cnt.wLeaves++;
					if (n != 0) {
						if (kLeafBatch == 1 && !FEWRAYS) soleFirst = nd[7];
						else if (laneNow() == 0) {
							LeafEntry en;
							en.first = nd[7]; en.count = n; en.maskLo = (uint32_t)m; en.maskHi = (uint32_t)(m >> 32); en.start = total; en.pad0 = en.pad1 = en.pad2 = 0;
							entries[batch] = en;
						}
						myReach |= pass ? 1u << batch : 0u;
						batch = uni(batch + 1);
						total = uni(total + n);
					}
				}
				nd = nxA;
				i = next;
			}
		}
		const uint32_t lane = laneNow();
		RTX_DBG_ONLY(
		const unsigned long long dbgP2 = __builtin_readcyclecounter();
		cnt.cNodes += dbgP2 - dbgP1;
		unsigned long long dbgExact = 0;
		)
		uint32_t ecur = 0;
		auto assign = [&](uint32_t p0, uint32_t& r, uint32_t& myEnt) {
			r = 0; myEnt = 0;
// ... 23 lines not shown
			if (RTX_DBG) { cnt.wTri += __popcll(cand); if (shadow) cnt.sExact += __popcll(cand); if (cand == 0) cnt.wS2++; }
			if (cand == 0) return false;
			bool improved = false;
			RTX_DBG_ONLY(const unsigned long long dbgE0 = __builtin_readcyclecounter();)
			if (FEWRAYS && !STATS && nRays4 <= (uint32_t)__popcll(cand) * 3u) {
				const uint64_t raysOpen = ballot(resume != kNever);
				const uint32_t mLo = entries[myEnt].maskLo, mHi = entries[myEnt].maskHi;
				const bool isCand = ((cand >> lane) & 1ull) != 0;
				uint64_t rays = raysOpen;
				while (rays != 0) {
					const int r = __builtin_ctzll(rays);
					rays &= rays - 1;
#define RTX_RL(x) __int_as_float(__builtin_amdgcn_readlane(__float_as_int(x), r))
					const float rox = RTX_RL(o.x), roy = RTX_RL(o.y), roz = RTX_RL(o.z), rdx = RTX_RL(d.x), rdy = RTX_RL(d.y), rdz = RTX_RL(d.z);
					const float rbt = RTX_RL(bt);
#undef RTX_RL
					const bool reached = ((((uint32_t)r & 32u) ? mHi : mLo) >> ((uint32_t)r & 31u)) & 1u;
					float t = __builtin_inff(), u = 0, v = 0;
					if (isCand && reached) triTestLane<CULL>(ra, rb, rc, rox, roy, roz, rdx, rdy, rdz, t, u, v);
					const bool better = t < rbt;
					const float tmin = -waveMax(better ? -t : -__builtin_inff());
					const uint64_t at = ballot(better && t == tmin);
					if (at != 0) {
						const int w = __builtin_ctzll(at);
						const float wt = __int_as_float(__builtin_amdgcn_readlane(__float_as_int(t), w)), wu = __int_as_float(__builtin_amdgcn_readlane(__float_as_int(u), w));
						const float wv = __int_as_float(__builtin_amdgcn_readlane(__float_as_int(v), w));
						const uint32_t wtri = (uint32_t)__builtin_amdgcn_readlane((int)ra.tri, w);
						if (lane == (uint32_t)r) { bt = wt; bu = wu; bv = wv; btri = wtri; improved = true; }
					}
				}
				cand = 0;
			}
			const float btBefore = bt;
			while (cand != 0) {
				const int c = __builtin_ctzll(cand);
				cand &= cand - 1;
#define RTX_RL(x) __int_as_float(__builtin_amdgcn_ds_bpermute(c << 2, __float_as_int(x)))
				const float v0x = RTX_RL(ra.v0x), v0y = RTX_RL(ra.v0y), v0z = RTX_RL(ra.v0z);
				const float e1x = RTX_RL(rb.e1x), e1y = RTX_RL(rb.e1y), e1z = RTX_RL(rb.e1z);
				const float e2x = RTX_RL(rb.e2x), e2y = RTX_RL(rc.e2y), e2z = RTX_RL(rc.e2z);
#undef RTX_RL
				const uint32_t tri = (uint32_t)__builtin_amdgcn_ds_bpermute(c << 2, (int)ra.tri);
				const uint32_t ent = (kLeafBatch == 1 && !FEWRAYS) ? 0u : (uint32_t)__builtin_amdgcn_ds_bpermute(c << 2, (int)myEnt);
				const bool pass = ((myReach >> ent) & 1u) != 0;
				if (pass) triTestOne<CULL, STATS>(v0x, v0y, v0z, e1x, e1y, e1z, e2x, e2y, e2z, tri, o, d, bt, bu, bv, btri);
			}
			improved = improved || bt < btBefore;
			RTX_DBG_ONLY(dbgExact += __builtin_readcyclecounter() - dbgE0;)
			if (ballot(improved) != 0) {
				if (!STATS) { if (shadow && bt < tLimit) resume = kNever; }
				const bool open = resume != kNever;
				tmaxB = unif(waveMax(open ? fminf(bt, tLimit) : -__builtin_inff()));
				if (!STATS && ballot(open) == 0) return true;
			}
			return false;
		};
		if (kLeafBatch == 1 && !FEWRAYS) {
			for (uint32_t p0 = 0; p0 < total; p0 = uni(p0 + 64)) {
				uint32_t rA, entA;
				assign(p0, rA, entA);
				const f4v vaA = *(const RTX_AS1 f4v*)(refA + (rA << 4)), vbA = *(const RTX_AS1 f4v*)(refB + (rA << 4));
				const f2v vcA = *(const RTX_AS1 f2v*)(refC + (rA << 3));
				if (process(p0, vaA, vbA, vcA, entA)) return;
			}
		}
		else
		for (uint32_t p0 = 0; p0 < total; p0 = uni(p0 + 128)) {
			uint32_t rA, entA, rB = 0, entB = 0;
			assign(p0, rA, entA);
			const f4v vaA = *(const RTX_AS1 f4v*)(refA + (rA << 4)), vbA = *(const RTX_AS1 f4v*)(refB + (rA << 4));
			const f2v vcA = *(const RTX_AS1 f2v*)(refC + (rA << 3));
			const bool two = p0 + 64 < total;
			if (two) assign(p0 + 64, rB, entB);
			const f4v vaB = *(const RTX_AS1 f4v*)(refA + (rB << 4)), vbB = *(const RTX_AS1 f4v*)(refB + (rB << 4));
			const f2v vcB = *(const RTX_AS1 f2v*)(refC + (rB << 3));
			if (process(p0, vaA, vbA, vcA, entA)) return;
			if (two && process(p0 + 64, vaB, vbB, vcB, entB)) return;
		}
		RTX_DBG_ONLY(cnt.cExact += dbgExact; cnt.cFilter += __builtin_readcyclecounter() - dbgP2 - dbgExact;)
		if (WIDE ? sp == 0 : i >= nN) break;
	}
}

template <bool STATS, bool MESH = true, bool FEWRAYS = false, bool BOXES = true, int CULLK = -1, int KINDS = 0, bool UNIO = false, bool LEAN = false>
__device__ __forceinline__ void traceWave(const Params& P, bool active, bool shadow, V3 o, V3 d, float tmax,
                                          Hit& h, Counts& cnt, uint32_t src = 0)
{
	h.obj = -1; h.t = tmax; h.tri = 0; h.u = 0; h.v = 0;
	if (STATS) cnt.rays += __popcll(ballot(active));
	const bool cull = CULLK < 0 ? (uni(P.view.flags) & 1u) != 0 : CULLK != 0;
	const float ix = 1 / d.x, iy = 1 / d.y, iz = 1 / d.z;
	const bool sx = LEAN ? false : ix < 0, sy = LEAN ? false : iy < 0, sz = LEAN ? false : iz < 0;
	bool live = active;
	const uint32_t nObj = uni(P.nObjects);
	for (uint32_t oi = 0; oi < nObj; oi = uni(oi + 1)) {
		const Object* ob = uni(P.objects + oi);
		const u32x16 rec = sload16(ob);
		const int type = (int)rec[0];
		const int mat = (int)rec[1];
		if (KINDS != 0 && (type == 3) != (KINDS == 2)) continue;
		const bool consider = live && !(shadow && mat == 2);
		if (ballot(consider) == 0) continue;
		if (MESH && type == 3) {
			const Mesh* M = uni(P.meshes + (int)rec[9]);
			const u32x16 rec2 = sload16((const char*)ob + 64);
			const u32x16 rec3 = sload16((const char*)ob + 128);
			const uint32_t mflags = rec2[13];
			bool pending = consider;
			const bool laneRegular = fabsf(ix) < __builtin_inff() && fabsf(iy) < __builtin_inff() && fabsf(iz) < __builtin_inff() &&
			                         fabsf(o.x) < 0x1p100f && fabsf(o.y) < 0x1p100f && fabsf(o.z) < 0x1p100f;
			const bool meshRegular0 = (mflags & 2u) != 0;
			const bool wideOk0 = (mflags & 4u) != 0;
			if ((mflags & 1u) != 0) {
				const float xlo = (F(rec2[2]) - o.x) * ix, xhi = (F(rec2[3]) - o.x) * ix, ylo = (F(rec2[4]) - o.y) * iy, yhi = (F(rec2[5]) - o.y) * iy;
				const float zlo = (F(rec2[6]) - o.z) * iz, zhi = (F(rec2[7]) - o.z) * iz;
				const bool bsx = LEAN ? negNow(ix) : sx, bsy = LEAN ? negNow(iy) : sy, bsz = LEAN ? negNow(iz) : sz;
				float tmin = bsx ? xhi : xlo, tmx = bsx ? xlo : xhi;
				const float tymin = bsy ? yhi : ylo, tymax = bsy ? ylo : yhi;
				bool fail = (tmin > tymax) || (tymin > tmx);
				if (tymin > tmin) tmin = tymin;
				if (tymax < tmx) tmx = tymax;
				const float tzmin = bsz ? zhi : zlo, tzmax = bsz ? zlo : zhi;
				fail = fail || (tmin > tzmax) || (tzmin > tmx);
				if (STATS) cnt.box += __popcll(ballot(consider && fail));
				pending = consider && !fail;
			}
			const bool oneOrigin0 = !STATS && ballot(pending && src != 1u) == 0;
			uint32_t fw = (mflags & 6u) | (oneOrigin0 ? 8u : 0u) | (ballot(pending && !laneRegular) != 0 ? 16u : 0u);
			while (ballot(pending) != 0) {
				bool cl = pending;
				uint32_t f = fw;
				if (LEAN) asm volatile("" : "+s"(f));
				const bool meshRegular = LEAN ? (f & 2u) != 0 : meshRegular0, wideOk = LEAN ? (f & 4u) != 0 : wideOk0, oneOrigin = (LEAN && !UNIO) ? (f & 8u) != 0 : oneOrigin0;
				bool regular = false;
				if (meshRegular) {
					bool lr = laneRegular;
					if (LEAN) {
						lr = true;
						if ((f & 16u) != 0) {
							lr = __builtin_amdgcn_inverse_ballot_w64(absBelowNow(ix, __builtin_inff()) & absBelowNow(iy, __builtin_inff()) & absBelowNow(iz, __builtin_inff()) &
							                                          absBelowNow(o.x, 0x1p100f) & absBelowNow(o.y, 0x1p100f) & absBelowNow(o.z, 0x1p100f));
						}
					}
					const uint64_t regM = ballot(pending && lr);
					if (regM != 0) { cl = pending && lr; regular = true; }
				}
				const char* ob2 = (const char*)ob + 96;
				asm volatile("" : "+s"(ob2));
				const u32x8 geo = sload8(ob2);
				const float fat = F(geo[0]), mcx = F(geo[1]), mcy = F(geo[2]), mcz = F(geo[3]), mrad = F(geo[4]);
				Bundle B = makeBundle(cl, o, d, oneOrigin);
				for (int split = 0; split < RTX_MAX_SPLITS; ++split) {
					const float dist = fmaxf(fmaxf(fabsf(B.ocx - mcx), fabsf(B.ocy - mcy)), fabsf(B.ocz - mcz)) + mrad;
					const float wo = B.roMax, wd = fmaxf(fmaxf(B.rdx, B.rdy), B.rdz) * dist;
					if (!(wo > fat || wd > fat)) break;
					bool lo;
					if (wo >= wd) lo = B.rox >= B.roy && B.rox >= B.roz ? o.x < B.ocx : (B.roy >= B.roz ? o.y < B.ocy : o.z < B.ocz);
					else lo = B.rdx >= B.rdy && B.rdx >= B.rdz ? d.x < B.dcx : (B.rdy >= B.rdz ? d.y < B.dcy : d.z < B.dcz);
					if (ballot(cl && lo) == 0 || ballot(cl && !lo) == 0) break;
					cl = cl && lo;
					B = makeBundle(cl, o, d, oneOrigin);
				}
				float bt, bu, bv; uint32_t btri;
				uint32_t srcSel = 0;
				if (!STATS) {
					const uint32_t s0 = (uint32_t)__builtin_amdgcn_readlane((int)src, __builtin_ctzll(ballot(cl)));
					if (s0 != 0) {
						const float l2 = len2(d);
						if (ballot(cl && !(src == s0 && l2 >= 0.9802f && l2 <= 1.002f)) == 0) srcSel = s0;
					}
				}
				V3 ow = o;
				if (UNIO) asm volatile("" : "+v"(ow.x), "+v"(ow.y), "+v"(ow.z));
				if (!STATS && cull && regular && wideOk) meshWalk<STATS, true, true, true, FEWRAYS, BOXES>(rec3, B, cl, shadow, ow, d, ix, iy, iz, sx, sy, sz, h.t, bt, bu, bv, btri, cnt, srcSel);
				else if (!STATS && regular && wideOk) meshWalk<STATS, false, true, true, FEWRAYS, BOXES>(rec3, B, cl, shadow, ow, d, ix, iy, iz, sx, sy, sz, h.t, bt, bu, bv, btri, cnt, srcSel);
				else if (cull && regular) meshWalk<STATS, true, true, false, FEWRAYS>(rec3, B, cl, shadow, ow, d, ix, iy, iz, sx, sy, sz, h.t, bt, bu, bv, btri, cnt);
				else if (cull) meshWalk<STATS, true, false, false, FEWRAYS>(rec3, B, cl, shadow, ow, d, ix, iy, iz, LEAN ? negNow(ix) : sx, LEAN ? negNow(iy) : sy, LEAN ? negNow(iz) : sz, h.t, bt, bu, bv, btri, cnt);
				else meshWalk<STATS, false, false, false, FEWRAYS>(rec3, B, cl, shadow, ow, d, ix, iy, iz, LEAN ? negNow(ix) : sx, LEAN ? negNow(iy) : sy, LEAN ? negNow(iz) : sz, h.t, bt, bu, bv, btri, cnt);
				if (cl && bt < kFltMax && bt < h.t) { h.obj = (int)oi; h.t = bt; h.tri = btri; h.u = bu; h.v = bv; }
				pending = pending && !cl;
			}
		}
		else {
			const V3 c = mk(F(rec[2]), F(rec[3]), F(rec[4]));
			float t0 = kFltMax; bool hit;
			if (type == 1) {
				const float r2 = F(rec[5]);
				const V3 L = c - o;
				const float tca = dot(L, d);
				const float d2 = dot(L, L) - tca * tca;
				hit = !(d2 > r2);
				const float thc = __builtin_sqrtf(r2 - d2);
				t0 = tca - thc;
				const float t1 = tca + thc;
				if (t0 < 0) t0 = t1;
				if (t0 < 0) hit = false;
			}
			else {
				const V3 n = mk(F(rec[6]), F(rec[7]), F(rec[8]));
				const float denom = dot(d, n);
				hit = !(fabsf(denom) < RTX_EPS8);
				t0 = dot(c - o, n) / denom;
				hit = hit && (t0 >= 0);
			}
			if (consider && hit && t0 < h.t) { h.obj = (int)oi; h.t = t0; h.u = 0; h.v = 0; }
		}
		if (!STATS) live = live && !(shadow && h.obj >= 0);
	}
}

enum : int {
	ST_DONE = 0, ST_NEWRAY, ST_WAIT_PRIMARY, ST_WAIT_SHADOW, ST_NEXT_LIGHT, ST_LIGHTS_DONE, ST_RETURN
};
enum : int { FR_REFL = 1, FR_TRANS1 = 2, FR_TRANS2 = 3 };

struct Lane {
	int state;
	int sp;
	V3 ro, rd;
	V3 col;
	int obj, mat;
	V3 P, N, objColor, diff, spec, L, I;
	float specCoef, nSpec, dsum, ssum;
	uint32_t li, si;
	float qtmax;
	bool qmoot;
	bool qarea;
	uint32_t qsrc;
};

__device__ __forceinline__ float& frameAt(const Params& P, uint32_t gl, int slot, int field)
{
	return P.frames[((size_t)slot * kFrameFields + field) * P.totalLanes + gl];
}

__device__ __forceinline__ void shadeObject(const Params& P, Lane& s, const Hit& h, const u32x16& a, const u32x16& b)
{
	s.mat = (int)a[1];
	s.objColor = mk(F(a[10]), F(a[11]), F(a[12]));
	s.specCoef = F(b[0]);
	s.nSpec = F(b[1]);
	const int type = (int)a[0];
	if (type == 1) s.N = normalized(s.P - mk(F(a[2]), F(a[3]), F(a[4])));
	else if (type == 2) s.N = mk(F(a[6]), F(a[7]), F(a[8]));
	else {
		const Mesh* M = uni(P.meshes + (int)a[9]);
		const GlobalFloats uvp = inGlobal((const float*)sloadp(&M->uv)) + (size_t)h.tri * 6;
		const GlobalFloats np = inGlobal((const float*)sloadp(&M->nrm)) + (size_t)h.tri * 9;
		const float* normalMap = (const float*)sloadp(&M->normal);
		const float* diffuseMap = (const float*)sloadp(&M->diffuse);
		const float* specularMap = (const float*)sloadp(&M->specular);
		const float u = h.u, v = h.v;
		const float w = 1 - u - v;
		const float texx = uvp[2] * u + uvp[4] * v + uvp[0] * w;
		const float texy = uvp[3] * u + uvp[5] * v + uvp[1] * w;
		V3 n = (load3(np + 3) * u + load3(np + 6) * v + load3(np) * (1 - u - v)) / 3;
		n = normalized(n);
		if (normalMap) {
			const GlobalFloats tbp = inGlobal((const float*)sloadp(&M->tb)) + (size_t)h.tri * 6;
			const uint32_t nW = sload1(&M->nW), nH = sload1(&M->nH);
			const int x = texel((int)nW, texx), y = texel((int)nH, texy);
			const V3 tn = normalized(load3(inGlobal(normalMap) + ((size_t)y * nW + x) * 3));
			V3 r;
			r.x = tn.x * tbp[0] + tn.y * tbp[3] + tn.z * n.x + 0.0f;
			r.y = tn.x * tbp[1] + tn.y * tbp[4] + tn.z * n.y + 0.0f;
			r.z = tn.x * tbp[2] + tn.y * tbp[5] + tn.z * n.z + 0.0f;
			n = normalized(r);
		}
		s.N = n;
		if (diffuseMap) {
			const uint32_t dW = sload1(&M->dW), dH = sload1(&M->dH);
			s.objColor = load3(inGlobal(diffuseMap) + ((size_t)texel((int)dH, texy) * dW + texel((int)dW, texx)) * 3);
		}
		if (specularMap) {
			const uint32_t sW = sload1(&M->sW), sH = sload1(&M->sH);
			s.specCoef = inGlobal(specularMap)[(size_t)texel((int)sH, texy) * sW + texel((int)sW, texx)];
		}
	}
}

__device__ __forceinline__ void shadePrimary(const Params& P, Lane& s, const Hit& h)
{
	s.obj = h.obj;
	s.P = s.ro + s.rd * h.t;
	for (uint64_t rem = ballot(true); rem != 0;) {
		const int o0 = __builtin_amdgcn_readlane(h.obj, __builtin_ctzll(rem));
		const Object* ob = uni(P.objects + o0);
		const u32x16 a = sload16(ob), b = sload16((const char*)ob + 64);
		const bool mine = h.obj == o0;
		if (mine) shadeObject(P, s, h, a, b);
		rem &= ~ballot(mine);
	}
	s.diff = mk(0, 0, 0); s.spec = mk(0, 0, 0);
	s.li = 0; s.si = 0; s.dsum = 0; s.ssum = 0;
}

struct LightRec { int type; V3 color; float intensity; V3 dir, pos; uint32_t nPoints; const float* points; };

template <bool PLAIN = false>
__device__ __forceinline__ void advance(const Params& P, Lane& s, uint32_t gl)
{
	const int maxDepth = P.view.maxDepth;
	const float bias = P.view.bias;
	V3& col = PLAIN ? s.diff : s.col;
	bool run = true;
	do {
		if (!run) continue;
		if (s.state == ST_NEWRAY) {
			RTX_T0
			if (s.sp > maxDepth) { col = skyColor(P, s.rd); s.state = ST_RETURN; RTX_ACC(0) continue; }
			s.qtmax = kFltMax;
			s.state = ST_WAIT_PRIMARY;
			run = false; continue;
		}
		if (s.state == ST_NEXT_LIGHT) {
			RTX_T0
			if (s.li >= P.nLights) { s.state = ST_LIGHTS_DONE; continue; }
			const uint32_t li0 = __builtin_amdgcn_readfirstlane(s.li);
			uint32_t liS = li0;
			if (PLAIN) asm volatile("" : "+s"(liS));
			if (s.li != li0) continue;
			LightRec lr;
			{
				const u32x16 w = sload16(P.lights + liS);
				lr.type = (int)w[0]; lr.color = mk(F(w[1]), F(w[2]), F(w[3])); lr.intensity = F(w[4]);
				lr.dir = mk(F(w[5]), F(w[6]), F(w[7])); lr.pos = mk(F(w[8]), F(w[9]), F(w[10])); lr.nPoints = w[11];
				lr.points = (const float*)(((uint64_t)w[13] << 32) | w[12]);
			}
			const LightRec* l = &lr;
			const int lt = l->type;
			if (PLAIN && lt != 1 && lt != 2) __builtin_unreachable();
			float dist;
			if (lt == 1) {
				s.L = l->dir;
				s.I = l->color * l->intensity;
				dist = kFltMax;
			}
			else if (lt == 2) {
				const V3 lp = l->pos;
				V3 L = s.P - lp;
				s.I = l->color * attenuation(l->intensity, len2(L));
				s.L = normalized(L);
				dist = length(s.P - lp);
			}
			else {
				const uint32_t np = l->nPoints;
				if (s.si == 0) {
					const V3 lp = l->pos;
					s.I = l->color * attenuation(l->intensity, len2(s.P - lp));
					s.dsum = 0; s.ssum = 0;
				}
				if (s.si >= np) {
					const float fn = (float)np;
					if (s.mat == 0) s.diff = s.diff + s.I * (s.dsum / fn);
					else if (s.mat == 3) {
						s.diff = s.diff + s.I * (s.dsum / fn);
						s.spec = s.spec + s.I * powfRef(s.ssum / fn, s.nSpec);
					}
					else s.spec = s.spec + s.I * powfRef(s.ssum / fn, s.nSpec);
					s.li++; s.si = 0;
					continue;
				}
				V3 L = s.P - load3(inGlobal(l->points) + (size_t)s.si * 3);
				dist = length(L);
				s.L = normalized(L);
			}
			s.qmoot = s.mat == 0 && fmaxRef(0.f, dot(s.N, -s.L)) == 0.f;
			s.qarea = lt == 3;
			s.qsrc = (lt == 2 && liS < P.nSrcLights && len2(s.N) <= P.srcNmax2) ? 2u + liS : 0u;
			s.qtmax = dist;
			s.state = ST_WAIT_SHADOW;
			RTX_ACC(1)
			run = false; continue;
		}
		if (s.state == ST_LIGHTS_DONE) {
			RTX_T0
			const Object* ob = P.objects + s.obj;
			if (PLAIN && s.mat != 0) __builtin_unreachable();
			if (s.mat == 0) { col = s.objColor * s.diff; s.state = ST_RETURN; continue; }
			if (s.mat == 3) {
				s.col = s.objColor * ob->ambient + s.diff * ob->diffuse + s.spec * s.specCoef;
				s.state = ST_RETURN; continue;
			}
			if (s.mat == 1) {
				frameAt(P, gl, s.sp, 0) = __int_as_float(FR_REFL);
				frameAt(P, gl, s.sp, 2) = s.spec.x; frameAt(P, gl, s.sp, 3) = s.spec.y; frameAt(P, gl, s.sp, 4) = s.spec.z;
				const V3 nd = s.rd - s.N * (2 * dot(s.rd, s.N));
				s.ro = s.P + s.N * bias; s.rd = nd;
				s.sp++; s.state = ST_NEWRAY; RTX_ACC(2) continue;
			}
			const float ior = ob->ior;
			const float kr = fresnelKr(s.rd, s.N, ior);
			const bool outside = dot(s.rd, s.N) < 0;
			const V3 biasVec = s.N * bias;
			const V3 fd = normalized(reflectDir(s.rd, s.N));
			const V3 fo = outside ? s.P + biasVec : s.P - biasVec;
			frameAt(P, gl, s.sp, 1) = kr;
			frameAt(P, gl, s.sp, 2) = s.spec.x; frameAt(P, gl, s.sp, 3) = s.spec.y; frameAt(P, gl, s.sp, 4) = s.spec.z;
			if (kr < 1) {
				const V3 rd = normalized(refractDir(s.rd, s.N, ior));
				const V3 ro = outside ? s.P - biasVec : s.P + biasVec;
				frameAt(P, gl, s.sp, 0) = __int_as_float(FR_TRANS1);
				frameAt(P, gl, s.sp, 8) = fo.x; frameAt(P, gl, s.sp, 9) = fo.y; frameAt(P, gl, s.sp, 10) = fo.z;
				frameAt(P, gl, s.sp, 11) = fd.x; frameAt(P, gl, s.sp, 12) = fd.y; frameAt(P, gl, s.sp, 13) = fd.z;
				s.ro = ro; s.rd = rd;
			}
			else {
				frameAt(P, gl, s.sp, 0) = __int_as_float(FR_TRANS2);
				frameAt(P, gl, s.sp, 5) = 0.f; frameAt(P, gl, s.sp, 6) = 0.f; frameAt(P, gl, s.sp, 7) = 0.f;
				s.ro = fo; s.rd = fd;
			}
			s.sp++; s.state = ST_NEWRAY; RTX_ACC(3) continue;
		}
		if (s.state == ST_RETURN) {
			RTX_T0
			if (s.sp == 0) { s.state = ST_DONE; run = false; continue; }
			if (PLAIN) __builtin_unreachable();
			s.sp--;
			float fr[kFrameFields];
			for (int k = 0; k < kFrameFields; ++k) fr[k] = frameAt(P, gl, s.sp, k);
			asm volatile("" : "+v"(fr[0]), "+v"(fr[1]), "+v"(fr[2]), "+v"(fr[3]), "+v"(fr[4]), "+v"(fr[5]), "+v"(fr[6]));
			asm volatile("" : "+v"(fr[7]), "+v"(fr[8]), "+v"(fr[9]), "+v"(fr[10]), "+v"(fr[11]), "+v"(fr[12]), "+v"(fr[13]));
			const int kind = __float_as_int(fr[0]);
			const V3 spec = mk(fr[2], fr[3], fr[4]);
			if (kind == FR_REFL) { s.col = s.col * 0.8f + spec; RTX_ACC(4) continue; }
			const float kr = fr[1];
			if (kind == FR_TRANS1) {
				const V3 acc = mk(0, 0, 0) + s.col * (1 - kr);
				frameAt(P, gl, s.sp, 0) = __int_as_float(FR_TRANS2);
				frameAt(P, gl, s.sp, 5) = acc.x; frameAt(P, gl, s.sp, 6) = acc.y; frameAt(P, gl, s.sp, 7) = acc.z;
				s.ro = mk(fr[8], fr[9], fr[10]);
				s.rd = mk(fr[11], fr[12], fr[13]);
// ... 14 lines not shown
{
	if (s.state == ST_WAIT_PRIMARY) {
		RTX_T0
		if (h.obj < 0) { (PLAIN ? s.diff : s.col) = skyColor(P, s.rd); s.state = ST_RETURN; RTX_ACC(7) return; }
		shadePrimary(P, s, h);
		if (PLAIN) s.mat = 0;
		s.state = ST_NEXT_LIGHT;
		RTX_ACC(8)
		return;
	}
	if (s.state == ST_WAIT_SHADOW) {
		RTX_T0
		const float vis = (h.obj < 0) ? 1.0f : 0.0f;
		if (PLAIN && (s.mat != 0 || s.qarea)) __builtin_unreachable();
		const bool area = s.qarea;
		const V3 nL = -s.L;
		if (s.mat == 0) {
			const float c = vis * fmaxRef(0.f, dot(s.N, nL));
			if (!area) s.diff = s.diff + s.I * c;
			else s.dsum += c;
		}
		else {
			const V3 R = reflectDir(s.L, s.N);
			const float sd = fmaxRef(0.f, dot(R, -s.rd));
			if (!area) {
				const V3 vI = s.I * vis;
				if (s.mat == 3) s.diff = s.diff + vI * fmaxRef(0.f, dot(s.N, nL));
				s.spec = s.spec + vI * powfRef(sd, s.nSpec);
			}
			else {
				if (s.mat == 3) s.dsum += vis * fmaxRef(0.f, dot(s.N, nL));
				s.ssum += vis * sd;
			}
		}
		if (area) s.si++; else s.li++;
		s.state = ST_NEXT_LIGHT;
		RTX_ACC(9)
	}
}

template <typename VIEW>
__device__ __forceinline__ void viewRay(const VIEW& view, float x, float y, V3& o, V3& d)
{
	const float w = (float)view.width, hgt = (float)view.height;
	const float xp = (2 * (x + 0.5f) / w - 1) * view.scale * view.aspect;
	const float yp = -(2 * (y + 0.5f) / hgt - 1) * view.scale;
	const V3 s = normalized(mk(xp, yp, -1));
	const float* M = view.camM;
	V3 r;
	r.x = s.x * M[0] + s.y * M[4] + s.z * M[8] + M[12];
	r.y = s.x * M[1] + s.y * M[5] + s.z * M[9] + M[13];
	r.z = s.x * M[2] + s.y * M[6] + s.z * M[10] + M[14];
	const float ww = s.x * M[3] + s.y * M[7] + s.z * M[11] + M[15];
	if (ww != 0.0f && ww != 1.0f) { const float wi = 1.0f / ww; r.x *= wi; r.y *= wi; r.z *= wi; }
	o = mk(view.camPos[0], view.camPos[1], view.camPos[2]);
	d = r;
}
__device__ __forceinline__ void primaryRay(const Params& P, float x, float y, V3& o, V3& d) { viewRay(P.view, x, y, o, d); }

constexpr int kParkFields = 25;
template <bool PLAIN> struct ParkLayout { static constexpr int kFields = kParkFields - (PLAIN ? 4 : 0), kSp = PLAIN ? -3 : 0; };
template <bool PLAIN>
__device__ __forceinline__ float (*parkArea())[256]
{
	__shared__ float area[ParkLayout<PLAIN>::kFields][256];
	return area;
}
static_assert(sizeof(powTab) + sizeof(leafBatch) + sizeof(wideStack) + sizeof(pruneUni) + ParkLayout<false>::kFields * 1024 <= (RTX_WAVES >= 5 ? 31744 : 40960),
              "the ray kernels' LDS no longer fits the blocks per CU that RTX_WAVES asks for");
static_assert(RTX_WAVES_PLAIN < 6 || sizeof(leafBatch) + sizeof(wideStack) + sizeof(pruneUni) + ParkLayout<true>::kFields * 1024 <= 27136,
              "the PLAIN kernels' LDS no longer fits six blocks per CU (160 KB / 6, rounded down to the allocation granule)");

__device__ __forceinline__ const Params& freshParams(const Params& P)
{
	uint64_t p = (uint64_t)(uintptr_t)__builtin_amdgcn_kernarg_segment_ptr();
	asm volatile("" : "+s"(p));
	return *(const Params*)(const RTX_AS4 Params*)p;
}

template <bool STATS, bool MESH = true, bool FEWRAYS = false, bool BOXES = true, bool CAM = true, int CULLK = -1, bool PLAIN = false>
__device__ __forceinline__ V3 castRayWave(const Params& P0, bool valid, V3 o, V3 d, uint32_t gl, Counts& cnt)
{
	const Params& P = freshParams(P0);
	Lane s;
	s.state = valid ? ST_NEWRAY : ST_DONE;
	s.sp = 0; s.ro = o; s.rd = d; s.col = mk(0, 0, 0);
	s.obj = 0; s.mat = 0; s.li = 0; s.si = 0;
	s.P = s.N = s.objColor = s.diff = s.spec = s.L = s.I = mk(0, 0, 0);
	s.specCoef = s.nSpec = s.dsum = s.ssum = 0;
	s.qtmax = kFltMax; s.qmoot = false; s.qarea = false; s.qsrc = 0;
	RTX_DBG_ONLY(unsigned long long dbgRounds = 0, dbgTrace = 0, dbgState = 0;)
	for (;;) {
		advance<PLAIN>(freshParams(P0), s, gl);
		if (ballot(s.state != ST_DONE) == 0) break;
		Hit h;
		RTX_DBG_ONLY(const unsigned long long dbgT0 = __builtin_readcyclecounter();)
		const bool moot = s.state == ST_WAIT_SHADOW && s.qmoot;
		if (STATS) cnt.moot += __popcll(ballot(moot));
		const bool qshadow = s.state == ST_WAIT_SHADOW;
		const V3 qo = qshadow ? s.P + s.N * P.view.bias : s.ro, qd = qshadow ? -s.L : s.rd;
		const bool qactive = s.state != ST_DONE && (STATS || !moot);
		const float qtmax = s.qtmax;
		const uint32_t qsrc = qshadow ? s.qsrc : ((CAM && s.sp == 0) ? 1u : 0u);
		if (MESH) { s.qtmax = kFltMax; s.qmoot = false; s.qsrc = 0; }
		if (MESH) {
			const uint32_t t = threadIdx.x;
			float (*parkedState)[256] = parkArea<PLAIN>();
			constexpr int kSp = ParkLayout<PLAIN>::kSp;
			parkedState[0][t] = s.P.x; parkedState[1][t] = s.P.y; parkedState[2][t] = s.P.z;
			parkedState[3][t] = s.N.x; parkedState[4][t] = s.N.y; parkedState[5][t] = s.N.z;
			parkedState[6][t] = s.objColor.x; parkedState[7][t] = s.objColor.y; parkedState[8][t] = s.objColor.z;
			parkedState[9][t] = s.diff.x; parkedState[10][t] = s.diff.y; parkedState[11][t] = s.diff.z;
			if (!PLAIN) { parkedState[12][t] = s.spec.x; parkedState[13][t] = s.spec.y; parkedState[14][t] = s.spec.z; }
			parkedState[15 + kSp][t] = s.L.x; parkedState[16 + kSp][t] = s.L.y; parkedState[17 + kSp][t] = s.L.z;
			parkedState[18 + kSp][t] = s.I.x; parkedState[19 + kSp][t] = s.I.y; parkedState[20 + kSp][t] = s.I.z;
			parkedState[21 + kSp][t] = s.rd.x; parkedState[22 + kSp][t] = s.rd.y; parkedState[23 + kSp][t] = s.rd.z;
			if (!PLAIN) parkedState[24][t] = s.specCoef;
			asm volatile("" ::: "memory");
		}
		traceWave<STATS, MESH, FEWRAYS, BOXES, CULLK>(freshParams(P0), qactive, qshadow, qo, qd, qtmax, h, cnt, qsrc);
		if (MESH) {
			asm volatile("" ::: "memory");
			const uint32_t t = threadIdx.x;
			float (*parkedState)[256] = parkArea<PLAIN>();
			constexpr int kSp = ParkLayout<PLAIN>::kSp;
			s.P = mk(parkedState[0][t], parkedState[1][t], parkedState[2][t]);
			s.N = mk(parkedState[3][t], parkedState[4][t], parkedState[5][t]);
			s.objColor = mk(parkedState[6][t], parkedState[7][t], parkedState[8][t]);
			s.diff = mk(parkedState[9][t], parkedState[10][t], parkedState[11][t]);
			if (!PLAIN) s.spec = mk(parkedState[12][t], parkedState[13][t], parkedState[14][t]);
			s.L = mk(parkedState[15 + kSp][t], parkedState[16 + kSp][t], parkedState[17 + kSp][t]);
			s.I = mk(parkedState[18 + kSp][t], parkedState[19 + kSp][t], parkedState[20 + kSp][t]);
			s.rd = mk(parkedState[21 + kSp][t], parkedState[22 + kSp][t], parkedState[23 + kSp][t]);
			if (!PLAIN) s.specCoef = parkedState[24][t];
		}
		RTX_DBG_ONLY(const unsigned long long dbgT1 = __builtin_readcyclecounter();)
		if (s.state != ST_DONE) {
			const Params& Pa = freshParams(P0);
			consume<PLAIN>(Pa, s, h);
		}
		RTX_DBG_ONLY(dbgRounds++; dbgTrace += dbgT1 - dbgT0; dbgState += __builtin_readcyclecounter() - dbgT1;)
	}
	RTX_DBG_ONLY(
	if (__lane_id() == 0) {
		const unsigned long long before = atomicMax(&gDbgHist[8], dbgTrace + dbgState);
		if (dbgTrace + dbgState > before) { gDbgHist[9] = dbgRounds; gDbgHist[10] = dbgTrace; gDbgHist[11] = dbgState; }
		atomicAdd(&gDbgHist[12], dbgRounds); atomicAdd(&gDbgHist[13], dbgTrace); atomicAdd(&gDbgHist[14], dbgState); atomicAdd(&gDbgHist[15], 1ull);
	}
	)
	return PLAIN ? s.diff : s.col;
}

constexpr int kParkFieldsPlainWave = 16;
__device__ __forceinline__ float (*parkAreaPlainWave())[256]
{
	__shared__ float area[kParkFieldsPlainWave][256];
	return area;
}
static_assert(RTX_WAVES_PLAIN < 6 || sizeof(leafBatch) + sizeof(wideStack) + sizeof(pruneUni) + kParkFieldsPlainWave * 1024 <= 27136,
              "the PLAIN pass-1 kernel's LDS no longer fits six blocks per CU");

template <bool STATS, bool FEWRAYS = false, bool BOXES = true, bool CAM = true, int CULLK = -1>
__device__ __forceinline__ V3 castRayPlainWave(const Params& P0, bool valid, V3 o, V3 d, uint32_t gl, Counts& cnt)
{
	static_assert(!STATS, "the instrumented kernels count moot rays and rounds: they keep the state machine (castRayWave)");
	const uint32_t t = threadIdx.x;
	float (*parked)[256] = parkAreaPlainWave();
	Lane s;
	s.diff = mk(0, 0, 0);
	if (freshParams(P0).view.maxDepth < 0) {
		if (valid) s.diff = skyColor(freshParams(P0), d);
		return s.diff;
	}
	constexpr bool SCALAR_STATE = CAM && !(BOXES && CULLK == 0);
	constexpr bool UNIO = SCALAR_STATE, LEAN = SCALAR_STATE;
	Hit h;
	parked[0][t] = d.x; parked[1][t] = d.y; parked[2][t] = d.z;
	if (!CAM) { parked[3][t] = o.x; parked[4][t] = o.y; parked[5][t] = o.z; }
	asm volatile("" ::: "memory");
	traceWave<STATS, true, FEWRAYS, BOXES, CULLK, 0, UNIO, LEAN>(freshParams(P0), valid, false, o, d, kFltMax, h, cnt, CAM ? 1u : 0u);
	asm volatile("" ::: "memory");
	const bool hit = h.obj >= 0;
	{
		const Params& P = freshParams(P0);
		s.rd = mk(parked[0][t], parked[1][t], parked[2][t]);
		s.ro = CAM ? mk(P.view.camPos[0], P.view.camPos[1], P.view.camPos[2]) : mk(parked[3][t], parked[4][t], parked[5][t]);
		if (valid && !hit) s.diff = skyColor(P, s.rd);
		if (ballot(hit) == 0) return s.diff;
		s.P = s.N = s.objColor = mk(0, 0, 0);
		if (hit) shadePrimary(P, s, h);
	}
	for (uint32_t li = 0; li < uni(freshParams(P0).nLights); li = uni(li + 1)) {
		V3 I; float m;
		{
			const Params& P = freshParams(P0);
			const u32x16 w = sload16(P.lights + li);
			const int lt = (int)w[0];
			const V3 lcolor = mk(F(w[1]), F(w[2]), F(w[3])); const float lint = F(w[4]);
			V3 L; float dist;
			if (lt == 1) {
				L = mk(F(w[5]), F(w[6]), F(w[7]));
				I = lcolor * lint;
				dist = kFltMax;
			}
			else {
				const V3 lp = mk(F(w[8]), F(w[9]), F(w[10]));
				const V3 Lv = s.P - lp;
				I = lcolor * attenuation(lint, len2(Lv));
				L = normalized(Lv);
				dist = length(s.P - lp);
			}
			const V3 nL = -L;
			m = fmaxRef(0.f, dot(s.N, nL));
			const bool active = hit && !(m == 0.f);
			h.obj = -1;
			if (ballot(active) != 0) {
				const uint32_t src = (lt == 2 && li < P.nSrcLights && len2(s.N) <= P.srcNmax2) ? 2u + li : 0u;
				const V3 so = s.P + s.N * P.view.bias;
				parked[0][t] = s.P.x; parked[1][t] = s.P.y; parked[2][t] = s.P.z;
				parked[3][t] = s.N.x; parked[4][t] = s.N.y; parked[5][t] = s.N.z;
				parked[6][t] = s.objColor.x; parked[7][t] = s.objColor.y; parked[8][t] = s.objColor.z;
				parked[9][t] = s.diff.x; parked[10][t] = s.diff.y; parked[11][t] = s.diff.z;
				parked[12][t] = I.x; parked[13][t] = I.y; parked[14][t] = I.z;
				parked[15][t] = m;
				asm volatile("" ::: "memory");
				traceWave<STATS, true, FEWRAYS, BOXES, CULLK, 0, false, LEAN>(freshParams(P0), active, true, so, nL, dist, h, cnt, src);
				asm volatile("" ::: "memory");
				s.P = mk(parked[0][t], parked[1][t], parked[2][t]);
				s.N = mk(parked[3][t], parked[4][t], parked[5][t]);
				s.objColor = mk(parked[6][t], parked[7][t], parked[8][t]);
				s.diff = mk(parked[9][t], parked[10][t], parked[11][t]);
				I = mk(parked[12][t], parked[13][t], parked[14][t]);
				m = parked[15][t];
			}
		}
		const float vis = (h.obj < 0) ? 1.0f : 0.0f;
		const float c = vis * m;
		if (hit) s.diff = s.diff + I * c;
	}
	return hit ? s.objColor * s.diff : s.diff;
}

__device__ __forceinline__ bool rowOwned(uint32_t bandH, uint32_t nParts, uint32_t part, uint32_t y)
{
	return bandH == 0 || (y / bandH) % nParts == part;
}
__device__ __forceinline__ bool rowRendered(const Params& P, uint32_t y)
{
	if (rowOwned(P.bandH, P.nParts, P.part, y)) return true;
	if (!P.halo) return false;
	return (y > 0 && rowOwned(P.bandH, P.nParts, P.part, y - 1)) || rowOwned(P.bandH, P.nParts, P.part, y + 1);
}

__device__ __forceinline__ uint32_t nextWork(uint32_t* counter)
{
	uint32_t w = 0;
	if (__lane_id() == 0) w = atomicAdd(counter, 1u);
	return __builtin_amdgcn_readfirstlane(w);
}

__device__ __forceinline__ void flushCounts(const Params& P, const Counts& c)
{
	if (__lane_id() == 0) {
		atomicAdd(P.counters + 0, c.rays);
		atomicAdd(P.counters + 1, c.box);
		atomicAdd(P.counters + 2, c.tri);
		atomicAdd(P.counters + 5, c.wNodes); atomicAdd(P.counters + 6, c.wTri); atomicAdd(P.counters + 7, c.wS2);
		atomicAdd(P.counters + 8, c.wS3); atomicAdd(P.counters + 9, c.wS4);
		atomicAdd(P.counters + 10, c.wLeaves); atomicAdd(P.counters + 11, c.wLeafSkips);
		atomicAdd(P.counters + 12, c.wChunks); atomicAdd(P.counters + 13, c.wChunkSkips); atomicAdd(P.counters + 14, c.triLanes);
		atomicAdd(P.counters + 15, c.moot);
		RTX_DBG_ONLY(
		atomicAdd(&gDbgHist[32], c.cNodes); atomicAdd(&gDbgHist[33], c.cFilter); atomicAdd(&gDbgHist[34], c.cExact);
		atomicAdd(&gDbgHist[40], c.aWalks); atomicAdd(&gDbgHist[41], c.sWalks); atomicAdd(&gDbgHist[42], c.sVisits); atomicAdd(&gDbgHist[43], c.sLeaves); atomicAdd(&gDbgHist[44], c.sPasses); atomicAdd(&gDbgHist[45], c.sExact);
		)
	}
}

}

template <bool STATS, bool MESH = true, bool BOXES = true, int CULLK = (STATS || !MESH) ? -1 : 1, bool PLAIN = false>
__global__ void __launch_bounds__(256, MESH ? (PLAIN ? RTX_WAVES_PLAIN : RTX_WAVES) : RTX_WAVES_ANALYTIC) rtxPass1Kernel(const Params P)
{
	if (!PLAIN) fillPowTab();
	const uint32_t gl = blockIdx.x * blockDim.x + threadIdx.x;
	const uint32_t lane = __lane_id();
	const uint32_t W = P.view.width, H = P.view.height;
	Counts cnt = {};
	const uint32_t xcd = __builtin_amdgcn_s_getreg((3 << 11) | (0 << 6) | 20) & 7u;
	RTX_TRACE_ONLY(
	const unsigned long long dbgStart = wall_clock64();
	unsigned long long dbgEnd = dbgStart, dbgBusy = 0;
	)
	for (uint32_t attempt = 0; attempt < 8; attempt = uni(attempt + 1)) {
		const uint32_t q = (xcd + attempt) & 7u;
		const uint32_t qBase = sload1(P.tileList + q), qSize = sload1(P.tileList + 8 + q);
		uint32_t take = 1, jEnd = 0, j = 0;
		for (;;) {
			if (j >= jEnd) {
				uint32_t w = 0;
				if (__lane_id() == 0) w = atomicAdd(P.workCounter + q * 16, take);
				j = __builtin_amdgcn_readfirstlane(w);
				if (j >= qSize) break;
				jEnd = j + take < qSize ? j + take : qSize;
				if (kPopDen * j >= kPopNum * qSize) take = RTX_POP_MANY;
			}
			const uint32_t tile = sload1(P.tileList + qBase + j);
			j = uni(j + 1);
			RTX_DBG_ONLY(if (P.pad3 != 0 && tile != P.pad3 - 1) continue;)
// ... 740 lines not shown
		while (todo) {
			const uint32_t l = (uint32_t)__builtin_ctzll(todo);
			todo &= todo - 1;
			const uint32_t n = (uint32_t)__builtin_amdgcn_readlane((int)nIdx, (int)l);
			const uint32_t ny = n / P.tilesXFull, nx = n - ny * P.tilesXFull;
			const uint64_t flags = frameSobelTile(P, nx, ny, lane);
			if (lane == 0) __hip_atomic_store(P.tileFlags + n, (unsigned long long)flags, RTX_AGENT);
			storesAcknowledged();
			uint32_t mIdx;
			uint64_t todo2 = ballot(frameCountIn(P, P.tileSobel, nx, ny, lane, mIdx));
			while (todo2) {
				const uint32_t l2 = (uint32_t)__builtin_ctzll(todo2);
				todo2 &= todo2 - 1;
				const uint32_t m = (uint32_t)__builtin_amdgcn_readlane((int)mIdx, (int)l2);
				const uint32_t nf = (uint32_t)__popcll(__hip_atomic_load(P.tileFlags + m, RTX_AGENT));
				uint32_t mode = 0, items = (nf + 15u) >> 4;
				if (items) {
					const uint32_t c = __hip_atomic_load(P.tileCost + m, RTX_AGENT);
					const uint32_t want = c > sload1(P.splitLimits + 1) ? 2u : (c > sload1(P.splitLimits) || c > RTX_SSAA_VERY * P.heavyTicks ? 1u : 0u);
					if (want) {
						const uint32_t spread = want == 2 ? nf : (nf + 3u) >> 2;
						uint32_t ok = 0;
						if (lane == 0) ok = atomicAdd(ctl + FC_VERY, spread - items) + (spread - items) <= P.veryBudget;
						if (__builtin_amdgcn_readfirstlane(ok)) { mode = want; items = spread; }
					}
				}
				if (items) {
					if (lane < items) {
						const uint32_t q = (rot + lane) & (RTX_FRAME_QUEUES - 1);
						const uint32_t slot = atomicAdd(ctl + FC_QUEUE + 16 * q + 1, 1u);
						if (slot >= P.queueCap) atomicExch(ctl + FC_ERROR, 3u);
						else __hip_atomic_store(P.ssaaQueue + (size_t)q * P.queueCap + slot, (unsigned long long)P.epoch << 32 | (m << 8 | lane << 2 | mode), RTX_AGENT);
					}
					rot = uni(rot + items);
					storesAcknowledged();
				}
				if (lane == 0) {
					const uint32_t k = m & 63u;
					if (atomicAdd(ctl + FC_COUNT + 16 * k, 1u) + 1 == P.countExpect[k] && atomicAdd(ctl + FC_GROUPS, 1u) + 1 == sload1(P.countExpect + 64))
						for (uint32_t r = 0; r < 64; ++r) __hip_atomic_store(ctl + FC_ALL + 16 * r, 1u, RTX_AGENT);
				}
			}
		}
	}
}

__global__ void __launch_bounds__(256) rtxQuantizeKernel(const float* __restrict__ fb, uint8_t* __restrict__ out,
                                                         uint32_t W, uint32_t H, uint32_t bandH, uint32_t nParts, uint32_t part)
{
	const size_t q = (size_t)blockIdx.x * blockDim.x + threadIdx.x;
	const uint32_t perRow = W / 4;
	if (q >= (size_t)perRow * H) return;
	const uint32_t row = (uint32_t)(q / perRow), x = (uint32_t)(q - (size_t)row * perRow) * 4;
	const uint32_t y = H - 1 - row;
	if (!rowOwned(bandH, nParts, part, y)) return;
	const float4* in = (const float4*)(fb + ((size_t)y * W + x) * 3);
	const float4 a = in[0], b = in[1], c = in[2];
	const float v[12] = { a.x, a.y, a.z, a.w, b.x, b.y, b.z, b.w, c.x, c.y, c.z, c.w };
	uint32_t o[3] = { 0, 0, 0 };
	for (int px = 0; px < 4; ++px)
		for (int k = 0; k < 3; ++k) {
			const uint32_t byte = (uint32_t)(uint8_t)(int)(clampRef(0.0f, 1.0f, v[px * 3 + (2 - k)]) * 255);
			const int at = px * 3 + k;
			o[at >> 2] |= byte << ((at & 3) * 8);
		}
	uint32_t* dst = (uint32_t*)(out + ((size_t)row * W + x) * 3);
	dst[0] = o[0]; dst[1] = o[1]; dst[2] = o[2];
}

__global__ void rtxMathProbeKernel(int op, uint32_t n, const float* x, const float* y, float* out)
{
	fillPowTab();
	const uint32_t i = blockIdx.x * blockDim.x + threadIdx.x;
	if (i >= n) return;
	float r = 0;
	if (op == 0) r = powfRef(x[i], y[i]);
	else if (op == 1) r = 1 / x[i];
	else if (op == 2) r = __builtin_sqrtf(x[i]);
	else if (op == 3) r = invLenD(x[i]);
	else if (op == 4) r = x[i] / y[i];
	out[i] = r;
}

__global__ void rtxVecProbeKernel(int op, uint32_t n, const float* a, const float* b, float ior, float* out)
{
	const uint32_t i = blockIdx.x * blockDim.x + threadIdx.x;
	if (i >= n) return;
	const V3 d = load3(a + (size_t)i * 3), nn = b ? load3(b + (size_t)i * 3) : mk(0, 0, 0);
	V3 r = mk(0, 0, 0);
	if (op == 0) r = reflectDir(d, nn);
	else if (op == 1) r = refractDir(d, nn, ior);
	else if (op == 2) r.x = fresnelKr(d, nn, ior);
	else if (op == 3) r = normalized(d);
	out[(size_t)i * 3] = r.x; out[(size_t)i * 3 + 1] = r.y; out[(size_t)i * 3 + 2] = r.z;
}

template __global__ void rtxPass1Kernel<false>(const Params);
template __global__ void rtxPass1Kernel<true>(const Params);
template __global__ void rtxSsaaKernel<false>(const Params);
template __global__ void rtxSsaaKernel<true>(const Params);
template __global__ void rtxPass1Kernel<false, false>(const Params);
template __global__ void rtxSsaaKernel<false, false>(const Params);
template __global__ void rtxFrameKernel<true>(const Params);
template __global__ void rtxFrameKernel<false>(const Params);
template __global__ void rtxPass1Kernel<false, true, false>(const Params);
template __global__ void rtxSsaaKernel<false, true, false>(const Params);
template __global__ void rtxFrameKernel<true, false>(const Params);
template __global__ void rtxPass1Kernel<false, true, true, 0>(const Params);
template __global__ void rtxPass1Kernel<false, true, false, 0>(const Params);
template __global__ void rtxSsaaKernel<false, true, true, 0>(const Params);
template __global__ void rtxSsaaKernel<false, true, false, 0>(const Params);
template __global__ void rtxFrameKernel<true, true, 0>(const Params);
template __global__ void rtxFrameKernel<true, false, 0>(const Params);
#define RTX_PLAIN_INSTANCES(B, C)                                                  \
template __global__ void rtxPass1Kernel<false, true, B, C, true>(const Params);    \
template __global__ void rtxSsaaKernel<false, true, B, C, true>(const Params);     \
template __global__ void rtxFrameKernel<true, B, C, true>(const Params);
RTX_PLAIN_INSTANCES(true, 1) RTX_PLAIN_INSTANCES(false, 1) RTX_PLAIN_INSTANCES(true, 0) RTX_PLAIN_INSTANCES(false, 0)
#undef RTX_PLAIN_INSTANCES

__device__ __forceinline__ V3 normalsCast(const Params& P, bool valid, V3 o, V3 d, uint32_t src, Hit& h)
{
	Counts cnt = {};
	traceWave<false, true, false, true, -1>(P, valid, false, o, d, kFltMax, h, cnt, src);
	V3 c = mk(0, 0, 0);
	if (!valid) return c;
	if (P.view.maxDepth < 0 || h.obj < 0) return skyColor(P, d);
	Lane s;
	s.ro = o; s.rd = d;
	shadePrimary(P, s, h);
	return s.N / 2.0f + mk(0.5f, 0.5f, 0.5f);
}

__global__ void __launch_bounds__(256) rtxNormalsKernel(const Params P, int mode)
{
	const uint32_t wave = blockIdx.x * 4 + (threadIdx.x >> 6), lane = __lane_id();
	const uint32_t W = P.view.width, H = P.view.height;
	Hit h;
	if (mode == 0) {
		if (wave >= P.nTiles) return;
		const uint32_t tx = wave % P.tilesX, ty = P.tileRow0 + wave / P.tilesX;
		const uint32_t x = tx * 8 + (lane & 7), y = ty * 8 + (lane >> 3);
		const bool valid = x < W - 1 && y < H - 1 && y >= P.rowBegin && y < P.rowEnd && rowRendered(P, y);
		if (ballot(valid) == 0) return;
		V3 o, d;
		primaryRay(P, (float)x + 0.5f, (float)y + 0.5f, o, d);
		const V3 c = normalsCast(P, valid, o, d, 1u, h);
		if (valid) { float* px = P.fb + ((size_t)y * W + x) * 3; px[0] = c.x; px[1] = c.y; px[2] = c.z; }
	}
	else if (mode == 1) {
		const size_t first = (size_t)P.rowBegin * W + (size_t)wave * 16, end = (size_t)P.rowEnd * W;
		if (first >= end) return;
		const size_t i = first + (lane >> 2);
		const uint32_t sub = lane & 3;
		const uint32_t y = (uint32_t)(i / W), x = (uint32_t)(i - (size_t)y * W);
		const bool valid = i < end && x < W - 1 && y < H - 1 && rowOwned(P.bandH, P.nParts, P.part, y) && P.ssaaMask[i] != 0;
		if (ballot(valid) == 0) return;
		const float fx = (float)x + ((sub & 2) ? 0.75f : 0.25f), fy = (float)y + ((sub & 1) ? 0.75f : 0.25f);
		V3 o, d;
		primaryRay(P, fx, fy, o, d);
		const V3 c = normalsCast(P, valid, o, d, 1u, h);
		const int base = (int)(lane & ~3u);
		V3 sum = mk(0, 0, 0);
		for (int k = 0; k < 4; ++k)
			sum = sum + mk(__shfl(c.x, base + k), __shfl(c.y, base + k), __shfl(c.z, base + k));
		if (valid && sub == 0) { float* px = P.fb + i * 3; px[0] = sum.x / 4; px[1] = sum.y / 4; px[2] = sum.z / 4; }
// ... 107 lines not shown
```

rendering_amd/csrc/rtx_light_loop.h:

```cpp
		const V3 O = p + n * P.view.bias;
		V3 diff = mk(0, 0, 0), spec = mk(0, 0, 0);
		const uint32_t nLights = uni(P.nLights);
		for (uint32_t li = 0; li < nLights; li = uni(li + 1)) {
			const u32x16 w = sload16(P.lights + li);
			const int lt = (int)w[0];
			const V3 lcolor = mk(F(w[1]), F(w[2]), F(w[3]));
			const float lint = F(w[4]);
			const V3 lpos = mk(F(w[8]), F(w[9]), F(w[10]));
			const bool area = lt == 3;
			const float* pts = (const float*)(((uint64_t)w[13] << 32) | w[12]);
			const uint32_t nPoints = w[11];
			const V3 I = lt == 1 ? lcolor * lint : lcolor * attenuation(lint, len2(p - lpos));
			float a = 0, b = 0;
			uint32_t nOpen = 0;
			const uint32_t nSamples = area ? nPoints : 1u;
			for (uint32_t k = 0; k < nSamples; k = uni(k + 1)) {
				V3 L;
				float dist;
				if (lt == 1) { L = mk(F(w[5]), F(w[6]), F(w[7])); dist = kFltMax; }
				else {
					V3 from = lpos;
					if (area) { const float* pk = uni(pts + (size_t)k * 3); from = mk(sloadf(pk), sloadf(pk + 1), sloadf(pk + 2)); }
					const V3 Lv = p - from;
					dist = length(Lv);
					L = normalized(Lv);
				}
				const V3 nL = -L;
				const float md = fmaxRef(0.f, dot(n, nL));
				const float sd = wantS ? fmaxRef(0.f, dot(reflectDir(L, n), -d)) : 0.f;
				bool moot;
				if (area) moot = (!wantD || md == 0.f) && (!wantS || sd == 0.f);
				else {
					a = md;
					if (wantS) b = powfRef(sd, ns);
					moot = (!wantD || plusZero(I * a)) && (!wantS || plusZero(I * b));
				}
				const bool lit = hit && (wantOpen || !moot);
				const bool asked = lit && !(dist != dist);
				bool open = asked;
				if (ballot(asked) != 0) {
					const float tmWalk = dist > kFltMax ? kFltMax : dist;
					if (!MESH) {
						traceWave<false, false, false, BOXES, CULLK>(P, open, true, O, nL, dist, h, cnt);
						open = open && h.obj < 0;
					}
					else {
						traceWave<false, false, false, BOXES, CULLK, 1>(P, open, true, O, nL, dist, h, cnt);
						open = open && h.obj < 0;
						if (ballot(open) != 0) {
							const uint32_t src = (lt == 2 && li < P.nSrcLights && len2(n) <= P.srcNmax2) ? 2u + li : 0u;
							traceWave<false, true, false, BOXES, CULLK, 2>(P, open, true, O, nL, tmWalk, h, cnt, src);
							open = open && h.obj < 0;
						}
					}
				}
				open = lit && (open || !asked);
				nOpen += open ? 1u : 0u;
				if (area) {
					const float vis = open ? 1.0f : 0.0f;
					a += vis * md;
					b += vis * sd;
				}
				else if (!open) { a = 0; b = 0; }
			}
			V3 D = mk(0, 0, 0), S = mk(0, 0, 0);
			if (area) {
				const float fn = (float)nPoints;
				if (hit && wantD) D = I * (a / fn);
				if (hit && wantS) S = I * powfRef(b / fn, ns);
			}
			else if (nOpen != 0) {
				if (wantD) D = I * a;
				if (wantS) S = I * b;
			}
			diff = diff + D; spec = spec + S;
			RTX_LIGHT_LOOP_PER_LIGHT
		}
#undef RTX_LIGHT_LOOP_PER_LIGHT
```

rendering_amd/csrc/rtx_tuning.h:

```cpp
#pragma once

#ifndef RTX_DBG
#define RTX_DBG 0
#endif
#ifndef RTX_WAVE_TRACE
#define RTX_WAVE_TRACE 0
#endif
#ifndef RTX_WAVES
#define RTX_WAVES 5
#endif
#ifndef RTX_WAVES_PLAIN
#define RTX_WAVES_PLAIN 6
#endif
#ifndef RTX_WAVES_SSAA
#define RTX_WAVES_SSAA 4
#endif
#ifndef RTX_WAVES_FRAME
#define RTX_WAVES_FRAME 4
#endif
#ifndef RTX_WAVES_ANALYTIC
#define RTX_WAVES_ANALYTIC 4
#endif
#ifndef RTX_POP_MANY
#define RTX_POP_MANY 4u
#endif
#ifndef RTX_PRIO_TICKS
#define RTX_PRIO_TICKS 50000u
#endif
#ifndef RTX_MAX_SPLITS
#define RTX_MAX_SPLITS 4
#endif
#ifndef RTX_LEAF_BATCH
#define RTX_LEAF_BATCH 1
#endif
#ifndef RTX_LEAF_BATCH_FEW
#define RTX_LEAF_BATCH_FEW 2
#endif
#ifndef RTX_SSAA_VERY
#define RTX_SSAA_VERY 2u
#endif
#ifndef RTX_SSAA_SPREAD_PX
#define RTX_SSAA_SPREAD_PX 4u
#endif
```

Baseline: 18400.

## Add fp32 attenuation fast path and packed-math slab test for wide BVH walk

Replaces the double-precision attenuation divide with an fp32 reciprocal plus Newton refinement, using host-precomputed hi/lo split constants stored in the light record's padding. It checks whether the result is provably correctly rounded and falls back to the fp64 divide when it cannot be sure. It also adds a packed v_pk_add/v_pk_mul slab test for the wide BVH node boxes, enabled by default only for the few-rays camera path. The aim is to cut fp64 throughput cost and VALU instruction count in box tests, at the price of more code complexity and register-pairing constraints.

```diff
diff --git a/include/rtx_debug.h b/include/rtx_debug.h
--- a/include/rtx_debug.h
+++ b/include/rtx_debug.h
@@ -41,6 +41,10 @@
 
 int rtx_math_probe(int device, int op, uint32_t n, const float* x, const float* y, float* out);
 
+int rtx_attenuation_words(float intensity, float* ah, float* al);
+
+int rtx_slab_probe(int device, uint32_t n_boxes, const float* boxes, const float* rays, float* out);
+
 int rtx_vec_probe(int device, int op, uint32_t n, const float* a, const float* b, float ior, float* out);
 
 int rtx_desc_serialize(const rtx_scene_desc* desc, void* out, size_t cap, size_t* need);
diff --git a/rendering_amd/__init__.py b/rendering_amd/__init__.py
--- a/rendering_amd/__init__.py
+++ b/rendering_amd/__init__.py
@@ -33,6 +33,7 @@
     "rtx_scene_lights_read", "rtx_scene_mesh_prune_copy_read", "rtx_scene_objects_read",
     "rtx_frame_mode_probe", "rtx_tile_list_probe", "rtx_place_probe",
     "rtx_views_plan_probe",
+    "rtx_attenuation_words", "rtx_slab_probe",
 ]
 
 RTX_EDIT_SYMBOLS = ["rtx_scene_set_object", "rtx_scene_update_mesh", "rtx_scene_set_lights", "rtx_scene_set_objects"]
@@ -157,6 +158,9 @@
     rtx.rtx_counters_read.argtypes = [vp, C.POINTER(Counters)]
     rtx.rtx_last_kernel_ms.argtypes = [vp, i32, C.POINTER(C.c_float)]
     rtx.rtx_math_probe.argtypes = [i32, i32, u32, vp, vp, vp]
+    if hasattr(rtx, "rtx_slab_probe"):
+        rtx.rtx_attenuation_words.argtypes = [C.c_float, C.POINTER(C.c_float), C.POINTER(C.c_float)]
+        rtx.rtx_slab_probe.argtypes = [i32, u32, vp, vp, vp]
     rtx.rtx_cast_rays.argtypes = [vp, u32, vp, vp, vp]
     rtx.rtx_trace_rays.argtypes = [vp, u32, vp, vp, vp, vp]
     rtx.rtx_occluded_rays.argtypes = [vp, u32, vp, vp, vp, vp]
@@ -543,6 +547,24 @@
     return out
 
 
+def attenuation_words(intensity):
+    rtx, _ = load()
+    ah, al = C.c_float(0), C.c_float(0)
+    _check(rtx.rtx_attenuation_words(C.c_float(float(intensity)), C.byref(ah), C.byref(al)), "rtx_attenuation_words")
+    return np.float32(ah.value), np.float32(al.value)
+
+
+def slab_probe(boxes, rays, device=0):
+    rtx, _ = load()
+    boxes = np.ascontiguousarray(boxes, np.float32)
+    rays = np.ascontiguousarray(rays, np.float32)
+    n = boxes.shape[0]
+    assert boxes.shape == (n, 8) and rays.shape == (n, 64, 6)
+    out = np.zeros((n, 64, 12), np.float32)
+    _check(rtx.rtx_slab_probe(device, n, _np_ptr(boxes), _np_ptr(rays), _np_ptr(out)), "rtx_slab_probe")
+    return out
+
+
 def vec_probe(op, a, b=None, ior=1.0, device=0):
     rtx, _ = load()
     a = np.ascontiguousarray(a, np.float32).reshape(-1, 3)
diff --git a/rendering_amd/csrc/rtx_api.hip b/rendering_amd/csrc/rtx_api.hip
--- a/rendering_amd/csrc/rtx_api.hip
+++ b/rendering_amd/csrc/rtx_api.hip
@@ -694,6 +694,9 @@
 		d.type = l.type; memcpy(d.color, l.color, 12); d.intensity = l.intensity;
 		memcpy(d.dir, l.dir, 12); memcpy(d.pos, l.pos, 12);
 		d.nPoints = l.n_points;
+		float ah, al;
+		attenuationWords(l.intensity, ah, al);
+		memcpy(&d.pad[0], &ah, 4); memcpy(&d.pad[1], &al, 4);
 		if (l.type == RTX_LIGHT_AREA) HIPCHK(bag.upload(l.points, (size_t)l.n_points * 3, &d.points));
 	}
 	HIPCHK(bag.upload(recs.data(), recs.size(), dev));
@@ -2218,7 +2221,7 @@
 
 int rtx_math_probe(int device, int op, uint32_t n, const float* x, const float* y, float* out)
 {
-	if (!x || !out || op < 0 || op > 4) return fail(RTX_ERR_ARG, "bad argument");
+	if (!x || !out || op < 0 || op > 6 || (op >= 5 && !y)) return fail(RTX_ERR_ARG, "bad argument");
 	int cnt = 0;
 	if (hipGetDeviceCount(&cnt) != hipSuccess || cnt <= 0) return fail(RTX_ERR_NO_DEVICE, "no HIP device visible");
 	HIPCHK(hipSetDevice(device));
@@ -2228,9 +2231,44 @@
 	HIPCHK(hipMemcpy(dx, x, bytes, hipMemcpyHostToDevice));
 	if (y) HIPCHK(hipMemcpy(dy, y, bytes, hipMemcpyHostToDevice));
 	else HIPCHK(hipMemset(dy, 0, bytes));
+	if (op >= 5) {
+		std::vector<float> ah(n), al(n);
+		for (uint32_t i = 0; i < n; i++) attenuationWords(y[i], ah[i], al[i]);
+		DevArray<float> dah, dal;
+		HIPCHK(dah.reserve(n)); HIPCHK(dal.reserve(n));
+		HIPCHK(hipMemcpy(dah, ah.data(), bytes, hipMemcpyHostToDevice)); HIPCHK(hipMemcpy(dal, al.data(), bytes, hipMemcpyHostToDevice));
+		hipLaunchKernelGGL(rtxAttenuationProbeKernel, dim3((n + 255) / 256), dim3(256), 0, nullptr, op, n, (const float*)dx, (const float*)dy, (const float*)dah, (const float*)dal, dout.get());
+		HIPCHK(hipGetLastError());
+		HIPCHK(hipMemcpy(out, dout, bytes, hipMemcpyDeviceToHost));
+		return RTX_OK;
+	}
 	hipLaunchKernelGGL(rtxMathProbeKernel, dim3((n + 255) / 256), dim3(256), 0, nullptr, op, n, (const float*)dx, (const float*)dy, dout.get());
 	HIPCHK(hipGetLastError());
 	HIPCHK(hipMemcpy(out, dout, bytes, hipMemcpyDeviceToHost));
+	return RTX_OK;
+}
+
+int rtx_attenuation_words(float intensity, float* ah, float* al)
+{
+	if (!ah || !al) return fail(RTX_ERR_ARG, "ah/al is NULL");
+	attenuationWords(intensity, *ah, *al);
+	return RTX_OK;
+}
+
+int rtx_slab_probe(int device, uint32_t n_boxes, const float* boxes, const float* rays, float* out)
+{
+	if (!boxes || !rays || !out || n_boxes == 0) return fail(RTX_ERR_ARG, "bad argument");
+	int cnt = 0;
+	if (hipGetDeviceCount(&cnt) != hipSuccess || cnt <= 0) return fail(RTX_ERR_NO_DEVICE, "no HIP device visible");
+	HIPCHK(hipSetDevice(device));
+	const size_t nb = (size_t)n_boxes * 8, nr = (size_t)n_boxes * 64 * 6, no = (size_t)n_boxes * 64 * 12;
+	DevArray<float> db, dr, dout;
+	HIPCHK(db.reserve(nb)); HIPCHK(dr.reserve(nr)); HIPCHK(dout.reserve(no));
+	HIPCHK(hipMemcpy(db, boxes, nb * sizeof(float), hipMemcpyHostToDevice));
+	HIPCHK(hipMemcpy(dr, rays, nr * sizeof(float), hipMemcpyHostToDevice));
+	hipLaunchKernelGGL(rtxSlabProbeKernel, dim3(n_boxes), dim3(64), 0, nullptr, n_boxes, (const float*)db, (const float*)dr, dout.get());
+	HIPCHK(hipGetLastError());
+	HIPCHK(hipMemcpy(out, dout, no * sizeof(float), hipMemcpyDeviceToHost));
 	return RTX_OK;
 }
 
diff --git a/rendering_amd/csrc/rtx_device.h b/rendering_amd/csrc/rtx_device.h
--- a/rendering_amd/csrc/rtx_device.h
+++ b/rendering_amd/csrc/rtx_device.h
@@ -83,6 +83,13 @@
 };
 static_assert(sizeof(Light) == 64, "light record = one 64-byte line");
 
+inline void attenuationWords(float intensity, float& ah, float& al)
+{
+	const double A = (double)intensity * 1000.0 / (4 * 3.14159265358979323846);
+	ah = (float)A;
+	al = (float)(A - (double)ah);
+}
+
 struct View {
 	uint32_t width, height;
 	float bias;
diff --git a/rendering_amd/csrc/rtx_kernels.hip b/rendering_amd/csrc/rtx_kernels.hip
--- a/rendering_amd/csrc/rtx_kernels.hip
+++ b/rendering_amd/csrc/rtx_kernels.hip
@@ -305,9 +305,27 @@
 
 __device__ __forceinline__ int texel(int dim, float coord) { int v = (int)(dim * coord); if (v >= dim) v = dim - 1; if (v < 0) v = 0; return v; }
 
-__device__ __forceinline__ float attenuation(float intensity, float l2)
-{
-	return fminRef(1.0f, (float)((double)intensity / (4 * 3.14159265358979323846 * (double)l2 / 1000)));
+__device__ __forceinline__ float attenuationSlow(float intensity, float l2) { return (float)((double)intensity / (4 * 3.14159265358979323846 * (double)l2 / 1000)); }
+__device__ __forceinline__ float attenuationFast(float l2, float ah, float al, bool& sure)
+{
+	const float y0 = __builtin_amdgcn_rcpf(l2);
+	const float q0 = ah * y0;
+	const float r0 = __builtin_fmaf(-q0, l2, ah) + al;
+	const float q1 = __builtin_fmaf(r0, y0, q0);
+	const float e = __builtin_fmaf(-q1, l2, ah) + al;
+	const uint32_t qb = __float_as_uint(q1);
+	const float ulp = __uint_as_float((qb & 0x7f800000u) - (23u << 23));
+	const bool inRange = qb - 0x2b800000u <= 0x53800000u - 0x2b800000u && __float_as_uint(l2) - 0x2b800000u <= 0x53800000u - 0x2b800000u;
+	sure = fabsf(e) < l2 * ulp * 0.49999237f && inRange && (qb & 0x007fffffu) != 0;
+	return q1;
+}
+__device__ __forceinline__ float attenuation(float intensity, float l2, float ah, float al)
+{
+	if (!RTX_ATTENUATION_FP32) return fminRef(1.0f, attenuationSlow(intensity, l2));
+	bool sure;
+	float r = attenuationFast(l2, ah, al, sure);
+	if (!sure) r = attenuationSlow(intensity, l2);
+	return fminRef(1.0f, r);
 }
 
 struct Hit { int obj; float t; uint32_t tri; float u, v; };
@@ -522,6 +540,34 @@
 	asm("v_min_f32 %0, %1, %2" : "=v"(nx) : "v"(xlo), "v"(xhi)); asm("v_max_f32 %0, %1, %2" : "=v"(fx) : "v"(xlo), "v"(xhi));
 	asm("v_min_f32 %0, %1, %2" : "=v"(ny) : "v"(ylo), "v"(yhi)); asm("v_max_f32 %0, %1, %2" : "=v"(fy) : "v"(ylo), "v"(yhi));
 	asm("v_min_f32 %0, %1, %2" : "=v"(nz) : "v"(zlo), "v"(zhi)); asm("v_max_f32 %0, %1, %2" : "=v"(fz) : "v"(zlo), "v"(zhi));
+	asm("v_max3_f32 %0, %1, %2, %3" : "=v"(tn) : "v"(nx), "v"(ny), "v"(nz));
+	asm("v_min3_f32 %0, %1, %2, %3" : "=v"(tf) : "v"(fx), "v"(fy), "v"(fz));
+	return tn > tf;
+}
+struct RayPairs { f2v x, y, z; };
+__device__ __forceinline__ RayPairs makeRayPairs(float ox, float oy, float oz, float ix, float iy, float iz)
+{
+	f2v x = f2v{ ox, ix }, y = f2v{ oy, iy }, z = f2v{ oz, iz };
+	asm volatile("" : "+v"(x), "+v"(y), "+v"(z));
+	RayPairs r;
+	r.x = x; r.y = y; r.z = z;
+	return r;
+}
+__device__ __forceinline__ f2v slabProductsPacked(uint32_t lo, uint32_t hi, f2v oi)
+{
+	const uint64_t box = ((uint64_t)hi << 32) | lo;
+	f2v d, p;
+	asm("v_pk_add_f32 %0, %1, %2 op_sel_hi:[1,0] neg_lo:[0,1] neg_hi:[0,1]" : "=v"(d) : "s"(box), "v"(oi));
+	asm("v_pk_mul_f32 %0, %1, %2 op_sel:[0,1] op_sel_hi:[1,1]" : "=v"(p) : "v"(d), "v"(oi));
+	return p;
+}
+__device__ __forceinline__ bool boxFailsPacked(uint32_t blox, uint32_t bhix, uint32_t bloy, uint32_t bhiy, uint32_t bloz, uint32_t bhiz, f2v rx, f2v ry, f2v rz)
+{
+	const f2v px = slabProductsPacked(blox, bhix, rx), py = slabProductsPacked(bloy, bhiy, ry), pz = slabProductsPacked(bloz, bhiz, rz);
+	float nx, ny, nz, fx, fy, fz, tn, tf;
+	asm("v_min_f32 %0, %1, %2" : "=v"(nx) : "v"(px.x), "v"(px.y)); asm("v_max_f32 %0, %1, %2" : "=v"(fx) : "v"(px.x), "v"(px.y));
+	asm("v_min_f32 %0, %1, %2" : "=v"(ny) : "v"(py.x), "v"(py.y)); asm("v_max_f32 %0, %1, %2" : "=v"(fy) : "v"(py.x), "v"(py.y));
+	asm("v_min_f32 %0, %1, %2" : "=v"(nz) : "v"(pz.x), "v"(pz.y)); asm("v_max_f32 %0, %1, %2" : "=v"(fz) : "v"(pz.x), "v"(pz.y));
 	asm("v_max3_f32 %0, %1, %2, %3" : "=v"(tn) : "v"(nx), "v"(ny), "v"(nz));
 	asm("v_min3_f32 %0, %1, %2, %3" : "=v"(tf) : "v"(fx), "v"(fy), "v"(fz));
 	return tn > tf;
@@ -603,11 +649,13 @@
 	return ~deadBits & 0x11111111u;
 }
 
-template <bool STATS, bool CULL, bool REGULAR, bool WIDE = false, bool FEWRAYS = false, bool BOXES = true>
+template <bool STATS, bool CULL, bool REGULAR, bool WIDE = false, bool FEWRAYS = false, bool BOXES = true, bool PACKED = false>
 __device__ __forceinline__ void meshWalk(const u32x16& mp, const Bundle& B, bool consider, bool shadow, const V3& o, const V3& d,
                                          float ix, float iy, float iz, bool sx, bool sy, bool sz, float tLimit,
-                                         float& bt, float& bu, float& bv, uint32_t& btri, Counts& cnt, uint32_t srcSel = 0)
-{
+                                         float& bt, float& bu, float& bv, uint32_t& btri, Counts& cnt, uint32_t srcSel = 0, f2v rpx = f2v{ 0, 0 }, f2v rpy = f2v{ 0, 0 }, f2v rpz = f2v{ 0, 0 })
+{
+	static_assert(!PACKED || WIDE, "only the wide walk's slot test has a packed form");
+
 #define RTX_MP(k) (((uint64_t)mp[2 * (k) + 1] << 32) | mp[2 * (k)])
 	const Node* nodes = (const Node*)RTX_MP(0);
 	const RTX_AS1 char* refA = (const RTX_AS1 char*)(uintptr_t)RTX_MP(1);
@@ -725,7 +773,8 @@
 #define RTX_ALIVE4(q) ((aliveM >> (16 * (q))) & 0x1111u)
 #define RTX_SLOT(rec, base, k)                                                                                                     \
 				if ((int32_t)rec[base + 6] != 0 && RTX_ALIVE(k)) {                                                         \
-					const bool fail = boxFailsRegular(F(rec[base]), F(rec[base + 1]), F(rec[base + 2]), F(rec[base + 3]), F(rec[base + 4]), F(rec[base + 5]), o, ix, iy, iz); \
+					const bool fail = PACKED ? boxFailsPacked(rec[base], rec[base + 1], rec[base + 2], rec[base + 3], rec[base + 4], rec[base + 5], rpx, rpy, rpz) \
+					                         : boxFailsRegular(F(rec[base]), F(rec[base + 1]), F(rec[base + 2]), F(rec[base + 3]), F(rec[base + 4]), F(rec[base + 5]), o, ix, iy, iz); \
 					const uint64_t mk_ = ballot(!fail) & inM;                                                                       \
 					if (RTX_DBG) cnt.wS3++;                                                                                         \
 					if (mk_ != 0) RTX_PUSH(rec[base + 6], rec[base + 7], mk_)                                                       \
@@ -744,7 +793,8 @@
 				if (RTX_ALIVE4(0) != 0) {
 					RTX_SLOT(wb, 8, 3) RTX_SLOT(wb, 0, 2) RTX_SLOT(wa, 8, 1)
 					if ((int32_t)wa[6] != 0 && RTX_ALIVE(0)) {
-						const bool fail = boxFailsRegular(F(wa[0]), F(wa[1]), F(wa[2]), F(wa[3]), F(wa[4]), F(wa[5]), o, ix, iy, iz);
+						const bool fail = PACKED ? boxFailsPacked(wa[0], wa[1], wa[2], wa[3], wa[4], wa[5], rpx, rpy, rpz)
+						                         : boxFailsRegular(F(wa[0]), F(wa[1]), F(wa[2]), F(wa[3]), F(wa[4]), F(wa[5]), o, ix, iy, iz);
 						const uint64_t mk_ = ballot(!fail) & inM;
 						if (RTX_DBG) cnt.wS3++;
 						if (mk_ != 0) {
@@ -934,14 +984,15 @@
 	}
 }
 
-template <bool STATS, bool MESH = true, bool FEWRAYS = false, bool BOXES = true, int CULLK = -1, int KINDS = 0, bool UNIO = false, bool LEAN = false>
-__device__ __forceinline__ void traceWave(const Params& P, bool active, bool shadow, V3 o, V3 d, float tmax,
+template <bool STATS, bool MESH = true, bool FEWRAYS = false, bool BOXES = true, int CULLK = -1, int KINDS = 0, bool UNIO = false, bool LEAN = false, bool PACKED = false>
+__device__ __forceinline__ void traceWave(const Params& P, bool active, bool shadow, V3 oIn, V3 d, float tmax,
                                           Hit& h, Counts& cnt, uint32_t src = 0)
 {
+	float ox = oIn.x, oy = oIn.y, oz = oIn.z;
 	h.obj = -1; h.t = tmax; h.tri = 0; h.u = 0; h.v = 0;
 	if (STATS) cnt.rays += __popcll(ballot(active));
 	const bool cull = CULLK < 0 ? (uni(P.view.flags) & 1u) != 0 : CULLK != 0;
-	const float ix = 1 / d.x, iy = 1 / d.y, iz = 1 / d.z;
+	float ix = 1 / d.x, iy = 1 / d.y, iz = 1 / d.z;
 	const bool sx = LEAN ? false : ix < 0, sy = LEAN ? false : iy < 0, sz = LEAN ? false : iz < 0;
 	bool live = active;
 	const uint32_t nObj = uni(P.nObjects);
@@ -950,6 +1001,7 @@
 		const u32x16 rec = sload16(ob);
 		const int type = (int)rec[0];
 		const int mat = (int)rec[1];
+		const V3 o = mk(ox, oy, oz);
 		if (KINDS != 0 && (type == 3) != (KINDS == 2)) continue;
 		const bool consider = live && !(shadow && mat == 2);
 		if (ballot(consider) == 0) continue;
@@ -981,6 +1033,7 @@
 			uint32_t fw = (mflags & 6u) | (oneOrigin0 ? 8u : 0u) | (ballot(pending && !laneRegular) != 0 ? 16u : 0u);
 			while (ballot(pending) != 0) {
 				bool cl = pending;
+				const V3 o = mk(ox, oy, oz);
 				uint32_t f = fw;
 				if (LEAN) asm volatile("" : "+s"(f));
 				const bool meshRegular = LEAN ? (f & 2u) != 0 : meshRegular0, wideOk = LEAN ? (f & 4u) != 0 : wideOk0, oneOrigin = (LEAN && !UNIO) ? (f & 8u) != 0 : oneOrigin0;
@@ -1023,9 +1076,16 @@
 					}
 				}
 				V3 ow = o;
-				if (UNIO) asm volatile("" : "+v"(ow.x), "+v"(ow.y), "+v"(ow.z));
-				if (!STATS && cull && regular && wideOk) meshWalk<STATS, true, true, true, FEWRAYS, BOXES>(rec3, B, cl, shadow, ow, d, ix, iy, iz, sx, sy, sz, h.t, bt, bu, bv, btri, cnt, srcSel);
-				else if (!STATS && regular && wideOk) meshWalk<STATS, false, true, true, FEWRAYS, BOXES>(rec3, B, cl, shadow, ow, d, ix, iy, iz, sx, sy, sz, h.t, bt, bu, bv, btri, cnt, srcSel);
+				RayPairs rp = { f2v{ 0, 0 }, f2v{ 0, 0 }, f2v{ 0, 0 } };
+				if (PACKED) {
+					rp = makeRayPairs(ox, oy, oz, ix, iy, iz);
+					ow.x = rp.x.x; ow.y = rp.y.x; ow.z = rp.z.x;
+					ix = rp.x.y; iy = rp.y.y; iz = rp.z.y;
+					if (!UNIO) { ox = rp.x.x; oy = rp.y.x; oz = rp.z.x; }
+				}
+				else if (UNIO) asm volatile("" : "+v"(ow.x), "+v"(ow.y), "+v"(ow.z));
+				if (!STATS && cull && regular && wideOk) meshWalk<STATS, true, true, true, FEWRAYS, BOXES, PACKED>(rec3, B, cl, shadow, ow, d, ix, iy, iz, sx, sy, sz, h.t, bt, bu, bv, btri, cnt, srcSel, rp.x, rp.y, rp.z);
+				else if (!STATS && regular && wideOk) meshWalk<STATS, false, true, true, FEWRAYS, BOXES, PACKED>(rec3, B, cl, shadow, ow, d, ix, iy, iz, sx, sy, sz, h.t, bt, bu, bv, btri, cnt, srcSel, rp.x, rp.y, rp.z);
 				else if (cull && regular) meshWalk<STATS, true, true, false, FEWRAYS>(rec3, B, cl, shadow, ow, d, ix, iy, iz, sx, sy, sz, h.t, bt, bu, bv, btri, cnt);
 				else if (cull) meshWalk<STATS, true, false, false, FEWRAYS>(rec3, B, cl, shadow, ow, d, ix, iy, iz, LEAN ? negNow(ix) : sx, LEAN ? negNow(iy) : sy, LEAN ? negNow(iz) : sz, h.t, bt, bu, bv, btri, cnt);
 				else meshWalk<STATS, false, false, false, FEWRAYS>(rec3, B, cl, shadow, ow, d, ix, iy, iz, LEAN ? negNow(ix) : sx, LEAN ? negNow(iy) : sy, LEAN ? negNow(iz) : sz, h.t, bt, bu, bv, btri, cnt);
@@ -1147,7 +1207,7 @@
 	s.li = 0; s.si = 0; s.dsum = 0; s.ssum = 0;
 }
 
-struct LightRec { int type; V3 color; float intensity; V3 dir, pos; uint32_t nPoints; const float* points; };
+struct LightRec { int type; V3 color; float intensity; V3 dir, pos; uint32_t nPoints; const float* points; float ah, al; };
 
 template <bool PLAIN = false>
 __device__ __forceinline__ void advance(const Params& P, Lane& s, uint32_t gl)
@@ -1178,6 +1238,7 @@
 				lr.type = (int)w[0]; lr.color = mk(F(w[1]), F(w[2]), F(w[3])); lr.intensity = F(w[4]);
 				lr.dir = mk(F(w[5]), F(w[6]), F(w[7])); lr.pos = mk(F(w[8]), F(w[9]), F(w[10])); lr.nPoints = w[11];
 				lr.points = (const float*)(((uint64_t)w[13] << 32) | w[12]);
+				lr.ah = F(w[14]); lr.al = F(w[15]);
 			}
 			const LightRec* l = &lr;
 			const int lt = l->type;
@@ -1191,7 +1252,7 @@
 			else if (lt == 2) {
 				const V3 lp = l->pos;
 				V3 L = s.P - lp;
-				s.I = l->color * attenuation(l->intensity, len2(L));
+				s.I = l->color * attenuation(l->intensity, len2(L), l->ah, l->al);
 				s.L = normalized(L);
 				dist = length(s.P - lp);
 			}
@@ -1199,7 +1260,7 @@
 				const uint32_t np = l->nPoints;
 				if (s.si == 0) {
 					const V3 lp = l->pos;
-					s.I = l->color * attenuation(l->intensity, len2(s.P - lp));
+					s.I = l->color * attenuation(l->intensity, len2(s.P - lp), l->ah, l->al);
 					s.dsum = 0; s.ssum = 0;
 				}
 				if (s.si >= np) {
@@ -1380,6 +1441,7 @@
 __device__ __forceinline__ V3 castRayWave(const Params& P0, bool valid, V3 o, V3 d, uint32_t gl, Counts& cnt)
 {
 	const Params& P = freshParams(P0);
+	constexpr bool kPackedSlab = CAM && MESH && !STATS && (FEWRAYS ? RTX_PACKED_FEW : RTX_PACKED_GENERAL) != 0;
 	Lane s;
 	s.state = valid ? ST_NEWRAY : ST_DONE;
 	s.sp = 0; s.ro = o; s.rd = d; s.col = mk(0, 0, 0);
@@ -1416,7 +1478,7 @@
 			if (!PLAIN) parkedState[24][t] = s.specCoef;
 			asm volatile("" ::: "memory");
 		}
-		traceWave<STATS, MESH, FEWRAYS, BOXES, CULLK>(freshParams(P0), qactive, qshadow, qo, qd, qtmax, h, cnt, qsrc);
+		traceWave<STATS, MESH, FEWRAYS, BOXES, CULLK, 0, false, false, kPackedSlab>(freshParams(P0), qactive, qshadow, qo, qd, qtmax, h, cnt, qsrc);
 		if (MESH) {
 			asm volatile("" ::: "memory");
 			const uint32_t t = threadIdx.x;
@@ -1472,11 +1534,12 @@
 	}
 	constexpr bool SCALAR_STATE = CAM && !(BOXES && CULLK == 0);
 	constexpr bool UNIO = SCALAR_STATE, LEAN = SCALAR_STATE;
+	constexpr bool PACKED = SCALAR_STATE && RTX_PACKED_PLAIN != 0;
 	Hit h;
 	parked[0][t] = d.x; parked[1][t] = d.y; parked[2][t] = d.z;
 	if (!CAM) { parked[3][t] = o.x; parked[4][t] = o.y; parked[5][t] = o.z; }
 	asm volatile("" ::: "memory");
-	traceWave<STATS, true, FEWRAYS, BOXES, CULLK, 0, UNIO, LEAN>(freshParams(P0), valid, false, o, d, kFltMax, h, cnt, CAM ? 1u : 0u);
+	traceWave<STATS, true, FEWRAYS, BOXES, CULLK, 0, UNIO, LEAN, PACKED>(freshParams(P0), valid, false, o, d, kFltMax, h, cnt, CAM ? 1u : 0u);
 	asm volatile("" ::: "memory");
 	const bool hit = h.obj >= 0;
 	{
@@ -1504,7 +1567,7 @@
 			else {
 				const V3 lp = mk(F(w[8]), F(w[9]), F(w[10]));
 				const V3 Lv = s.P - lp;
-				I = lcolor * attenuation(lint, len2(Lv));
+				I = lcolor * attenuation(lint, len2(Lv), F(w[14]), F(w[15]));
 				L = normalized(Lv);
 				dist = length(s.P - lp);
 			}
@@ -1522,7 +1585,7 @@
 				parked[12][t] = I.x; parked[13][t] = I.y; parked[14][t] = I.z;
 				parked[15][t] = m;
 				asm volatile("" ::: "memory");
-				traceWave<STATS, true, FEWRAYS, BOXES, CULLK, 0, false, LEAN>(freshParams(P0), active, true, so, nL, dist, h, cnt, src);
+				traceWave<STATS, true, FEWRAYS, BOXES, CULLK, 0, false, LEAN, PACKED>(freshParams(P0), active, true, so, nL, dist, h, cnt, src);
 				asm volatile("" ::: "memory");
 				s.P = mk(parked[0][t], parked[1][t], parked[2][t]);
 				s.N = mk(parked[3][t], parked[4][t], parked[5][t]);
@@ -2429,6 +2492,30 @@
 	out[i] = r;
 }
 
+__global__ void rtxAttenuationProbeKernel(int op, uint32_t n, const float* l2, const float* intensity, const float* ah, const float* al, float* out)
+{
+	const uint32_t i = blockIdx.x * blockDim.x + threadIdx.x;
+	if (i >= n) return;
+	if (op == 5) out[i] = attenuation(intensity[i], l2[i], ah[i], al[i]);
+	else { bool sure; attenuationFast(l2[i], ah[i], al[i], sure); out[i] = sure ? 0.0f : 1.0f; }
+}
+
+__global__ void __launch_bounds__(64) rtxSlabProbeKernel(uint32_t nBoxes, const float* boxes, const float* rays, float* out)
+{
+	const uint32_t b = blockIdx.x;
+	if (b >= nBoxes) return;
+	const u32x8 bx = sload8(boxes + (size_t)b * 8);
+	const size_t i = (size_t)b * 64 + threadIdx.x;
+	const V3 o = load3(rays + i * 6);
+	const float ix = rays[i * 6 + 3], iy = rays[i * 6 + 4], iz = rays[i * 6 + 5];
+	float* dst = out + i * 12;
+	dst[0] = (F(bx[0]) - o.x) * ix; dst[1] = (F(bx[1]) - o.x) * ix; dst[2] = (F(bx[2]) - o.y) * iy; dst[3] = (F(bx[3]) - o.y) * iy;
+	dst[4] = (F(bx[4]) - o.z) * iz; dst[5] = (F(bx[5]) - o.z) * iz;
+	const RayPairs rp = makeRayPairs(o.x, o.y, o.z, ix, iy, iz);
+	const f2v px = slabProductsPacked(bx[0], bx[1], rp.x), py = slabProductsPacked(bx[2], bx[3], rp.y), pz = slabProductsPacked(bx[4], bx[5], rp.z);
+	dst[6] = px.x; dst[7] = px.y; dst[8] = py.x; dst[9] = py.y; dst[10] = pz.x; dst[11] = pz.y;
+}
+
 __global__ void rtxVecProbeKernel(int op, uint32_t n, const float* a, const float* b, float ior, float* out)
 {
 	const uint32_t i = blockIdx.x * blockDim.x + threadIdx.x;
diff --git a/rendering_amd/csrc/rtx_light_loop.h b/rendering_amd/csrc/rtx_light_loop.h
--- a/rendering_amd/csrc/rtx_light_loop.h
+++ b/rendering_amd/csrc/rtx_light_loop.h
@@ -10,7 +10,7 @@
 			const bool area = lt == 3;
 			const float* pts = (const float*)(((uint64_t)w[13] << 32) | w[12]);
 			const uint32_t nPoints = w[11];
-			const V3 I = lt == 1 ? lcolor * lint : lcolor * attenuation(lint, len2(p - lpos));
+			const V3 I = lt == 1 ? lcolor * lint : lcolor * attenuation(lint, len2(p - lpos), F(w[14]), F(w[15]));
 			float a = 0, b = 0;
 			uint32_t nOpen = 0;
 			const uint32_t nSamples = area ? nPoints : 1u;
diff --git a/rendering_amd/csrc/rtx_tuning.h b/rendering_amd/csrc/rtx_tuning.h
--- a/rendering_amd/csrc/rtx_tuning.h
+++ b/rendering_amd/csrc/rtx_tuning.h
@@ -21,6 +21,18 @@
 #ifndef RTX_WAVES_ANALYTIC
 #define RTX_WAVES_ANALYTIC 4
 #endif
+#ifndef RTX_PACKED_PLAIN
+#define RTX_PACKED_PLAIN 0
+#endif
+#ifndef RTX_PACKED_GENERAL
+#define RTX_PACKED_GENERAL 0
+#endif
+#ifndef RTX_PACKED_FEW
+#define RTX_PACKED_FEW 1
+#endif
+#ifndef RTX_ATTENUATION_FP32
+#define RTX_ATTENUATION_FP32 1
+#endif
 #ifndef RTX_POP_MANY
 #define RTX_POP_MANY 4u
 #endif
```

Result: no change. 18480, median of 6 (+0.4%).
